# latteine1217/NSFnet

Hardware: AMD Instinct MI355X
Metric: collocation-pt NS-residual evals/sec, Re=2000 6x256 MLP (higher is better)
Workload: dtype bf16x3 (bf16 MFMA, hi/lo split, f32 accumulate)

## Files before the change

nsfnet_amd/csrc/balance.hip:

```cpp
#include <cmath>

#include "kernels.h"

namespace {

constexpr int kBlk = 64;
constexpr int kUpdThreads = 256;

__device__ __forceinline__ void wave_abs_stats(float v, double& mx, double& sm) {
  const double a = fabs((double)v);
  mx = wave_fold<FoldNanMax>(a);
  sm = wave_fold<FoldSum>(a);
}

__global__ __launch_bounds__(512) void reduce_terms_kernel(TermReduceArgs a) {
  __shared__ double part[3][8][64];
  const int H = a.H, HP = a.HP, L = a.L;
  const size_t P = flat_total(H, L, a.n_out);
  const int lane = threadIdx.x & 63, w = threadIdx.x >> 6;
  const size_t p = blockIdx.x * (size_t)64 + lane;
  const bool live = p < P;
  const ReduceLoc loc = live ? reduce_locate(p, H, HP, L, a.n_out) : ReduceLoc{-1, -1, 0};
  const size_t SG = sg_total(HP, L);
  int k = 0;
  for (int t = 0; t < 3; ++t) {
    double s = 0.0;
    for (int j = 0; j < a.nsrc[t]; ++j, ++k)
      if (live) s = reduce_source_add(s, a.src[k], loc, HP, SG, w);
    part[t][w][lane] = s;
  }
  __syncthreads();
  if (w != 0) return;
  float vt[3];
  for (int t = 0; t < 3; ++t) {
    float v = 0.f;
    if (a.out[t] && live) {
      double s = part[t][0][lane];
#pragma unroll
      for (int i = 1; i < 8; ++i) s += part[t][i][lane];
      v = (a.acc_mask >> t) & 1 ? a.out[t][p] + (float)s : (float)s;
      a.out[t][p] = v;
    }
    if (a.partials) {
      double mx, sm;
      wave_abs_stats(v, mx, sm);
      if (lane == 0) {
        a.partials[(size_t)blockIdx.x * 6 + 2 * t] = mx;
        a.partials[(size_t)blockIdx.x * 6 + 2 * t + 1] = sm;
      }
    }
    vt[t] = v;
  }
  if (a.gram) wave_gram(vt[0], vt[1], vt[2], lane, a.gram + (size_t)blockIdx.x * 6);
}

__global__ __launch_bounds__(64) void balance_stats_kernel(const float* __restrict__ v0, const float* __restrict__ v1,
                                                           const float* __restrict__ v2, long n,
                                                           double* __restrict__ partials) {
  const long p = blockIdx.x * (long)kBlk + threadIdx.x;
  const float* v[3] = {v0, v1, v2};
  for (int t = 0; t < 3; ++t) {
    double mx, sm;
    wave_abs_stats(v[t] && p < n ? v[t][p] : 0.f, mx, sm);
    if (threadIdx.x == 0) {
      partials[(size_t)blockIdx.x * 6 + 2 * t] = mx;
      partials[(size_t)blockIdx.x * 6 + 2 * t + 1] = sm;
    }
  }
}

__global__ __launch_bounds__(kUpdThreads) void balance_update_kernel(const double* __restrict__ partials, long nblk,
                                                                     long n, int terms, double beta,
                                                                     float* __restrict__ lam, double* record) {
  __shared__ double red[kUpdThreads][6];
  const int tid = threadIdx.x;
  strided_tree_fold<kUpdThreads, FoldNanMax, FoldSum, FoldNanMax, FoldSum, FoldNanMax, FoldSum>(
      [&](long b, int c) { return partials[b * 6 + c]; }, nblk, red);
  if (tid != 0) return;
  const double P = (double)n;
  const double max_r = red[0][0];
  double rec[12];
  for (int c = 0; c < 12; ++c) rec[c] = record[c];
  rec[0] = max_r; rec[1] = red[0][1] / P;
  for (int t = 1; t < 3; ++t) {
    const int base = 2 + 3 * (t - 1);
    const double mean = red[0][2 * t + 1] / P;
    rec[base] = red[0][2 * t]; rec[base + 1] = mean;
    if (!((terms >> (t - 1)) & 1)) { rec[base + 2] = 0.0; continue; }
    const double lhat = max_r / mean;
    rec[base + 2] = lhat;
    if (mean == 0.0 || !isfinite(lhat)) { rec[8] += 1.0; continue; }
    rec[8 + t] = (1.0 - beta) * rec[8 + t] + beta * lhat;
  }
  rec[11] += 1.0;
  for (int c = 0; c < 12; ++c) record[c] = rec[c];
  lam[0] = (float)rec[9];
  lam[1] = (float)rec[10];
}

__global__ void balance_combine_kernel(float* g, const float* gr, const float* __restrict__ gb,
                                       const float* __restrict__ gs, const float* __restrict__ lam, long n) {
  const float lb = lam[0], ls = gs ? lam[1] : 0.f;
  for (long i = blockIdx.x * (long)blockDim.x + threadIdx.x; i < n; i += (long)gridDim.x * blockDim.x) {
    float v = fmaf(lb, gb[i], gr[i]);
    if (gs) v = fmaf(ls, gs[i], v);
    g[i] = v;
  }
}

}

long balance_blocks(long n) { return (n + kBlk - 1) / kBlk; }

int launch_reduce_terms(const TermReduceArgs& a, hipStream_t s) {
  size_t P = flat_total(a.H, a.L, a.n_out);
  hipLaunchKernelGGL(reduce_terms_kernel, dim3((unsigned)((P + 63) / 64)), dim3(512), 0, s, a);
  return launch_status();
}

int launch_balance_stats(const float* v0, const float* v1, const float* v2, long n, double* partials, hipStream_t s) {
  hipLaunchKernelGGL(balance_stats_kernel, dim3((unsigned)balance_blocks(n)), dim3(kBlk), 0, s, v0, v1, v2, n, partials);
  return launch_status();
}

int launch_balance_update(const double* partials, long n, int terms, double beta, float* lam, double* record,
                          hipStream_t s) {
  hipLaunchKernelGGL(balance_update_kernel, dim3(1), dim3(kUpdThreads), 0, s, partials, balance_blocks(n), n, terms,
                     beta, lam, record);
  return launch_status();
}

int launch_balance_combine(float* g, const float* gr, const float* gb, const float* gs, const float* lam, long n,
                           hipStream_t s) {
  int blocks = (int)((n + 255) / 256);
  if (blocks > 2048) blocks = 2048;
  hipLaunchKernelGGL(balance_combine_kernel, dim3(blocks), dim3(256), 0, s, g, gr, gb, gs, lam, n);
  return launch_status();
}
```

nsfnet_amd/csrc/bwd_bf16_split.hip:

```cpp
#include "kernels.h"
#include "point_stage.h"
#include "split_phases.h"

template <int HP>
struct SplitBwdLds {
  using XI = XImg<HP, 32>;
  static constexpr size_t X_BYTES = XI::BYTES;
  static constexpr size_t OADJ_F = (size_t)2 * 4 * 128;
  static constexpr size_t DUMMY_F = 64 * 8;
  static size_t bytes(int L) { return X_BYTES + (OADJ_F + DUMMY_F + 6 * HP + (size_t)sg_total(HP, L)) * sizeof(float); }
};

template <int HP, int TERMS>
__global__ __launch_bounds__(2 * HP, 1) void bwd_split_kernel(BwdArgs a) {
  using G = SplitBwdLds<HP>;
  using SW = SplitWave<HP, TERMS>;
  constexpr int GT = HP, PPL = SW::PPL, COLS = SW::COLS;
  extern __shared__ __attribute__((aligned(16))) unsigned char ldsb[];
  float* const oadjL = reinterpret_cast<float*>(ldsb + G::X_BYTES);
  float* const dummy = oadjL + G::OADJ_F;
  float* const woutL = dummy + G::DUMMY_F;
  float* const w0L = woutL + 3 * HP;
  float* const sgacc = w0L + 3 * HP;
  const int tid = threadIdx.x, lane0 = tid & 63;
  const int wave = __builtin_amdgcn_readfirstlane(tid >> 6);
  const int grp = wave >> 2, w = wave & 3;
  const int gtid = tid - grp * GT;
  const float* __restrict__ P = a.prep;
  const int L = a.L;
  const int npad = a.ntiles * PPL;
  const int SG = sg_total(HP, L);
  float* const oadjG = oadjL + (size_t)grp * 4 * 128;
  for (int i = tid; i < SG; i += 2 * GT) sgacc[i] = 0.f;
  for (int i = tid; i < 3 * HP; i += 2 * GT) { woutL[i] = P[prep_wout(HP, L) + i]; w0L[i] = P[prep_w0x(HP) + i]; }
  for (int i = tid; i < (int)G::DUMMY_F; i += 2 * GT) dummy[i] = 0.f;
  float dbo[3] = {0.f, 0.f, 0.f};
  SW sw(ldsb, P, woutL, w0L, w, lane0);

  auto S_of = [&](int tile, int l) { return a.S + spill_off<act_block(HP, COLS)>(a.spill, tile < a.ntiles ? tile : 0, l, L); };
  auto Z_of = [&](int tile, int l) { return a.Zb + spill_off<act_block(HP, COLS)>(a.spill, tile, l, L); };
  auto seeds = [&](int tile, float& px, float& py) {
    const int col = lane0 & 31;
    if (tile < a.ntiles) {
      float pxa[1], pya[1];
      output_adjoint_stage<PPL, COLS, 4, GT, 1>(a, tile, gtid, col, col, npad, oadjG, dbo, pxa, pya);
      px = pxa[0]; py = pya[0];
    } else {
      for (int i = gtid; i < 3 * COLS; i += GT) oadjG[i] = 0.f;
      px = py = 0.f;
    }
  };
  auto oadj = [&](int col, int, float (&oc)[3][4]) {
#pragma unroll
    for (int c = 0; c < 3; ++c)
#pragma unroll
      for (int s = 0; s < 4; ++s) oc[c][s] = oadjG[c * COLS + s * PPL + col];
  };
  auto none = [](auto&&...) {};

  const int npairs = (a.ntiles + 1) / 2;
  float px = 0.f, py = 0.f, pxN = 0.f, pyN = 0.f;
  if ((int)blockIdx.x < npairs) seeds(2 * (int)blockIdx.x + grp, px, py);
  __syncthreads();
  if (grp == 1) SW::idle();
  for (int pair = blockIdx.x; pair < npairs; pair += gridDim.x) {
    const int tile = 2 * pair + grp;
    const int next_tile = pair + (int)gridDim.x < npairs ? 2 * (pair + (int)gridDim.x) + grp : -1;
    sw.template bphase<0, false>(L - 1, L, S_of(tile, L - 1), Z_of(tile, L - 1), px, py, sgacc, dummy + wave * 64, oadj, none);
    for (int l = L - 1; l >= 2; --l) {
      sw.template mphase<true, true>(l, S_of(tile, l - 1));
      sw.template bphase<1, false>(l - 1, L, S_of(tile, l - 1), Z_of(tile, l - 1), px, py, sgacc, dummy + wave * 64, oadj, none);
    }
    sw.template mphase<true, false>(1, nullptr);
    sw.template bphase<2, false>(0, L, S_of(tile, 0), Z_of(tile, 0), px, py, sgacc, dummy + wave * 64, oadj,
                                 [&](int q) { if (q == 3 && next_tile >= 0) seeds(next_tile, pxN, pyN); });
    px = pxN; py = pyN;
  }
  if (grp == 0) SW::idle();
  float* red = reinterpret_cast<float*>(ldsb);
  __syncthreads();
#pragma unroll
  for (int c = 0; c < 3; ++c) red[c * 2 * GT + tid] = dbo[c];
  __syncthreads();
  if (tid < 3) {
    float s = 0.f;
    for (int t = 0; t < 2 * GT; ++t) s += red[tid * 2 * GT + t];
    sgacc[sg_bout(HP, L) + tid] = s;
  }
  __syncthreads();
  float* out = a.sg + (size_t)blockIdx.x * SG;
  for (int i = tid; i < SG; i += 2 * GT) out[i] = sgacc[i];
}

size_t bwd_split_lds_bytes(int HP, int L) { (void)HP; return SplitBwdLds<256>::bytes(L); }

template <int HP, int TERMS>
static int launch_one(const BwdArgs& a, int grid, hipStream_t s) {
  const size_t lds = SplitBwdLds<HP>::bytes(a.L);
  if (!spill_is(a.spill, act_block(HP), IN_P24_COMPACT)) return -1000;
  return launch_or_configure(&bwd_split_kernel<HP, TERMS>, dim3(grid), dim3(2 * HP), lds, s, a.configure, a);
}

int launch_bwd_split(int HP, int terms, const BwdArgs& a, int grid, hipStream_t s) {
  if (HP != 256) return -1000;
  return terms == 3 ? launch_one<256, 3>(a, grid, s) : launch_one<256, 1>(a, grid, s);
}
```

nsfnet_amd/csrc/capi.hip:

```cpp
#include <cmath>
#include <cstdio>
#include <cstring>
#include <cstdlib>
#include <new>

#include "../../include/nsfnet_pinn.h"
#include "kernels.h"
#include "optim.h"
#include "rwf.h"

static_assert((int)PINN_FLD_COUNT == (int)FLD_COUNT, "field plane enum mismatch");

static thread_local char g_err[512] = "";
static int fail(int code, const char* fmt, const char* a = "", long b = 0) {
  snprintf(g_err, sizeof(g_err), fmt, a, b);
  return code;
}
static int hipfail(int rc, const char* what) {
  if (rc == -1000) return fail(-22, "%s: unsupported hidden width or spill layout (code %ld)", what, (long)rc);
  return fail(rc, "%s: HIP error %ld", what, (long)-rc);
}

struct Switches {
  int sched_f, sched_b;
  int wsplit, fuse;
  int stagger;
  int s0_skip32;
  int verbose;
  int tile_cols;
};
static int env_int(const char* name, int dflt) {
  const char* v = getenv(name);
  return v ? atoi(v) : dflt;
}
static Switches read_switches() {
  const int sched = env_int("PINN_SCHED", 2);
  return {env_int("PINN_FWD_SCHED", sched), env_int("PINN_BWD_SCHED", sched), env_int("PINN_WSPLIT", 1),
          env_int("PINN_FUSE", 1), env_int("PINN_STAGGER", 0), env_int("PINN_S0_SKIP32", 1),
          env_int("PINN_VERBOSE", 0), env_int("PINN_TILE_COLS", 0)};
}

struct pinn_net_s {
  int n_out, L, H, HP;
  int wide;
  int prec_fwd, prec_bwd, prec_dw;
};
static int terms_of(int prec) { return prec == 1 ? 3 : 1; }
static int pick_wide(const pinn_net_s* n) {
  if (n->HP > 256) return 1;
  if (n->HP != 256 && n->HP != 128) return 0;
  const bool fp32 = !n->prec_fwd && !n->prec_bwd && !n->prec_dw;
  const int force = read_switches().tile_cols;
  if (force == 64) return 1;
  if (force == 128) return 0;
  return fp32 && n->HP == 256;
}

enum Family { FAM_NONE = 0, FAM_FP32, FAM_FP32_WIDE, FAM_BF16, FAM_BF16_WIDE, FAM_PIPE, FAM_SPLIT, FAM_WSPLIT, FAM_FUSED };
static constexpr const char* FAMILY_NAMES[][3] = {
    {nullptr, nullptr, nullptr},
    {"fwd_kernel", "bwd_kernel", "dw_kernel"},
    {"fwd_wide_kernel", "bwd_wide_kernel", "dw_wide_kernel"},
    {"fwd_bf16_kernel", "bwd_bf16_kernel", "dw_bf16_kernel"},
    {"fwd_bf16_wide_kernel", "bwd_bf16_wide_kernel", "dw_bf16_wide_kernel"},
    {"fwd_pipe_kernel", "bwd_pipe_kernel", nullptr},
    {"fwd_split_kernel", "bwd_split_kernel", nullptr},
    {"fwd_wsplit_kernel", "bwd_wsplit_kernel", nullptr},
    {"fwdbwd_split_kernel", "fwdbwd_split_kernel", nullptr},
};
static constexpr unsigned FAMILY_SPILLS[][3] = {
    {0, 0, 0},
    {IN_CLASSIC | IN_SKIP0, IN_CLASSIC | IN_SKIP0, IN_CLASSIC | IN_SKIP0},
    {IN_CLASSIC | IN_SKIP0, IN_CLASSIC | IN_SKIP0, IN_CLASSIC | IN_SKIP0},
    {IN_CLASSIC, IN_CLASSIC, IN_CLASSIC | IN_P24_COMPACT},
    {IN_CLASSIC | IN_P24_WIDE, IN_CLASSIC | IN_P24_WIDE, IN_CLASSIC | IN_P24_WIDE},
    {IN_CLASSIC, IN_CLASSIC, 0},
    {IN_P24_COMPACT, IN_P24_COMPACT, 0},
    {IN_P24_WIDE, IN_P24_WIDE, 0},
    {IN_P24_COMPACT, IN_P24_COMPACT, 0},
};
static Family base_family(const pinn_net_s& n, int prec) {
  return prec ? (n.HP > 256 ? FAM_BF16_WIDE : FAM_BF16) : n.wide ? FAM_FP32_WIDE : FAM_FP32;
}

enum { ROLE_FWD_SAVE = 0, ROLE_FWD, ROLE_BWD, ROLE_DW, ROLE_FUSED, ROLE_COUNT };
static constexpr int ROLE_SPILL_COL[ROLE_COUNT] = {0, -1, 1, 2, 0};
struct Role {
  Family family;
  int grid;
  size_t lds;
  const char* name;
};

struct pinn_plan_s {
  pinn_net_s net;
  long n;
  int streams, ntiles, npad;
  int groups;
  int stagger;
  Role role[ROLE_COUNT];
  Spill spill;
  HardBc hbc;
  size_t off_partials, off_oadj, off_sg, off_slabs, off_S, off_Zb, bytes_fwd, bytes_all;
};

static int num_cus() {
  int dev = 0, n = 0;
  if (hipGetDevice(&dev) == hipSuccess &&
      hipDeviceGetAttribute(&n, hipDeviceAttributeMultiprocessorCount, dev) == hipSuccess && n > 0)
    return n;
  (void)hipGetLastError();
  return 256;
}

static size_t align_up(size_t v, size_t a) { return (v + a - 1) / a * a; }

static size_t fwd_lds(Family f, const pinn_net_s& n) {
  switch (f) {
    case FAM_FP32: return fwd_lds_bytes(n.HP);
    case FAM_FP32_WIDE: return fwd_wide_lds_bytes(n.HP);
    case FAM_BF16: return fwd_bf16_lds_bytes(n.HP, n.L, n.wide ? 64 : 128);
    case FAM_BF16_WIDE: return fwd_bf16_wide_lds_bytes(n.HP, n.L);
    case FAM_PIPE: return fwd_pipe_lds_bytes(n.HP, n.L);
    case FAM_SPLIT: return fwd_split_lds_bytes(n.HP, n.L);
    case FAM_WSPLIT: return fwd_wsplit_lds_bytes(n.HP);
    default: return 0;
  }
}
static size_t bwd_lds(Family f, const pinn_net_s& n) {
  switch (f) {
    case FAM_FP32: return bwd_lds_bytes(n.HP, n.L);
    case FAM_FP32_WIDE: return bwd_wide_lds_bytes(n.HP, n.L);
    case FAM_BF16: return bwd_bf16_lds_bytes(n.HP, n.L, n.wide ? 64 : 128);
    case FAM_BF16_WIDE: return bwd_bf16_wide_lds_bytes(n.HP, n.L);
    case FAM_PIPE: return bwd_pipe_lds_bytes(n.HP, n.L);
    case FAM_SPLIT: return bwd_split_lds_bytes(n.HP, n.L);
    case FAM_WSPLIT: return bwd_wsplit_lds_bytes(n.HP, n.L);
    default: return 0;
  }
}
static size_t dw_lds(Family f, const pinn_net_s& n) {
  switch (f) {
    case FAM_FP32: return dw_lds_bytes(n.HP);
    case FAM_FP32_WIDE: return dw_wide_lds_bytes();
    case FAM_BF16: return dw_bf16_lds_bytes(n.HP);
    case FAM_BF16_WIDE: return dw_bf16_wide_lds_bytes();
    default: return 0;
  }
}
static int run_fwd(const pinn_plan_s* plan, const Role& r, const FwdArgs& a, hipStream_t s) {
  const pinn_net_s& n = plan->net;
  const int NS = plan->streams, terms = terms_of(n.prec_fwd);
  switch (r.family) {
    case FAM_FP32: return launch_fwd(n.HP, NS, a, r.grid, s);
    case FAM_FP32_WIDE: return launch_fwd_wide(n.HP, NS, a, r.grid, s);
    case FAM_BF16: return launch_fwd_bf16(n.HP, NS, terms, n.wide ? 64 : 128, a, r.grid, s);
    case FAM_BF16_WIDE: return launch_fwd_bf16_wide(n.HP, NS, terms, a, r.grid, s);
    case FAM_PIPE: return launch_fwd_pipe(n.HP, terms, a, r.grid, s);
    case FAM_SPLIT: return launch_fwd_split(n.HP, terms, a, r.grid, s);
    case FAM_WSPLIT: return launch_fwd_wsplit(n.HP, terms, a, r.grid, s);
    default: return -1000;
  }
}
static int run_bwd(const pinn_plan_s* plan, const BwdArgs& a, hipStream_t s) {
  const pinn_net_s& n = plan->net;
  const Role& r = plan->role[ROLE_BWD];
  const int NS = plan->streams, terms = terms_of(n.prec_bwd);
  switch (r.family) {
    case FAM_FP32: return launch_bwd(n.HP, NS, a, r.grid, s);
    case FAM_FP32_WIDE: return launch_bwd_wide(n.HP, NS, a, r.grid, s);
    case FAM_BF16: return launch_bwd_bf16(n.HP, NS, terms, n.wide ? 64 : 128, a, r.grid, s);
    case FAM_BF16_WIDE: return launch_bwd_bf16_wide(n.HP, NS, terms, a, r.grid, s);
    case FAM_PIPE: return launch_bwd_pipe(n.HP, terms, a, r.grid, s);
    case FAM_SPLIT: return launch_bwd_split(n.HP, terms, a, r.grid, s);
    case FAM_WSPLIT: return launch_bwd_wsplit(n.HP, terms, a, r.grid, s);
    default: return -1000;
  }
}
static int run_dw(const pinn_plan_s* plan, const DwArgs& d, hipStream_t s) {
  const pinn_net_s& n = plan->net;
  const int NS = plan->streams, terms = terms_of(n.prec_dw);
  switch (plan->role[ROLE_DW].family) {
    case FAM_FP32: return launch_dw(n.HP, NS, d, s);
    case FAM_FP32_WIDE: return launch_dw_wide(n.HP, NS, d, s);
    case FAM_BF16: return launch_dw_bf16(n.HP, NS, terms, n.wide ? 64 : 128, d, s);
    case FAM_BF16_WIDE: return launch_dw_bf16_wide(n.HP, NS, terms, d, s);
    default: return -1000;
  }
}
static int run_fused(const pinn_plan_s* plan, const FwdArgs& fa, const BwdArgs& ba, hipStream_t s) {
  return launch_fwdbwd_split(plan->net.HP, terms_of(plan->net.prec_fwd), fa, ba, plan->role[ROLE_FUSED].grid, s);
}

static int resolve_plan(pinn_plan_s* p, const pinn_net_s& net, long n_points, int streams, int cus, const Switches& sw_in,
                        const HardBc& hbc = HardBc{}) {
  Switches sw = sw_in;
  if (hbc.kind) { sw.sched_f = sw.sched_b = 0; sw.wsplit = 0; sw.fuse = 0; }
  p->net = net;
  p->hbc = hbc;
  p->n = n_points; p->streams = streams;
  const bool wide = net.wide != 0;
  const int per_tile = wide ? (streams == 4 ? 16 : 64) : (streams == 4 ? 32 : 128);
  p->ntiles = (int)((n_points + per_tile - 1) / per_tile);
  p->npad = p->ntiles * per_tile;
  const int HP = net.HP, L = net.L, NW = HP / 32;
  auto bpc = [&](size_t lds) {
    int b = (int)(PINN_LDS_MAX / lds);
    int bw = NW >= 8 ? (wide && NW == 8 ? 2 : 1) : 8 / NW;
    if (b > bw) b = bw;
    return b < 1 ? 1 : b;
  };
  auto role = [&](int which, Family f, int grid, size_t lds, int name_col) {
    p->role[which] = Role{f, grid, lds, FAMILY_NAMES[f][name_col]};
  };
  const Family f8 = base_family(net, net.prec_fwd), b8 = base_family(net, net.prec_bwd), d8 = base_family(net, net.prec_dw);
  const size_t lds_f = fwd_lds(f8, net), lds_b = bwd_lds(b8, net), lds_d = dw_lds(d8, net);
  if (lds_b > PINN_LDS_MAX || lds_f > PINN_LDS_MAX) return fail(-22, "pinn_plan_create: this depth x width needs more than 160 KiB of LDS%s");
  int grid_f = cus * bpc(lds_f);
  if (grid_f > p->ntiles) grid_f = p->ntiles;
  int grid_b = cus * bpc(lds_b);
  if (grid_b > p->ntiles) grid_b = p->ntiles;
  const int grid_fp = cus < (p->ntiles + 1) / 2 ? cus : (p->ntiles + 1) / 2;
  const bool pipe_shape = HP == 256 && !wide && streams == 4 && L >= 2;
  int sf = sw.sched_f, sb = sw.sched_b;
  if (!pipe_shape || !net.prec_fwd) sf = 0;
  if (!pipe_shape || !net.prec_bwd) sb = 0;
  if (sf == 2 && fwd_lds(FAM_SPLIT, net) > PINN_LDS_MAX) sf = 1;
  if (sf == 1 && fwd_lds(FAM_PIPE, net) > PINN_LDS_MAX) sf = 0;
  if (sb == 2 && bwd_lds(FAM_SPLIT, net) > PINN_LDS_MAX) sb = 1;
  if (sb == 1 && bwd_lds(FAM_PIPE, net) > PINN_LDS_MAX) sb = 0;
  if (sf < 0 || sf > 2) sf = 0;
  if (sb < 0 || sb > 2) sb = 0;
  const bool split_pair = sf == 2 && sb == 2 && net.prec_dw;
  if (!split_pair) { if (sf == 2) sf = 1; if (sb == 2) sb = 1; }
  const bool s24w = HP > 256 && streams == 4 && net.prec_fwd && net.prec_bwd && net.prec_dw;
  const bool wsplit = s24w && L >= 2 && sw.wsplit != 0 && fwd_lds(FAM_WSPLIT, net) <= PINN_LDS_MAX &&
                      bwd_lds(FAM_WSPLIT, net) <= PINN_LDS_MAX;
  const bool fuse = sf == 2 && sb == 2 && split_pair && net.prec_fwd == net.prec_bwd && sw.fuse != 0 &&
                    fwdbwd_split_lds_bytes(HP, L) <= PINN_LDS_MAX;
  p->stagger = sw.stagger;
  if (sw.verbose)
    fprintf(stderr, "[pinn] plan: %ld pts, %d streams, HP %d, L %d, prec %d/%d/%d, wide %d, schedule fwd %d bwd %d\n",
            (long)n_points, streams, HP, L, net.prec_fwd, net.prec_bwd, net.prec_dw, (int)wide, sf, sb);
  if (sw.verbose && hbc.kind)
    fprintf(stderr, "[pinn] plan: hard wall conditions, lid-driven cavity at (%g, %g) x %g, lift power %d, lid sharpness %g\n",
            (double)hbc.x0, (double)hbc.y0, (double)hbc.inv_len, hbc.m, (double)hbc.r);
  const Family fs = wsplit ? FAM_WSPLIT : sf == 2 ? FAM_SPLIT : sf == 1 ? FAM_PIPE : f8;
  const Family bs = wsplit ? FAM_WSPLIT : sb == 2 ? FAM_SPLIT : sb == 1 ? FAM_PIPE : b8;
  role(ROLE_FWD, f8, grid_f, lds_f, 0);
  role(ROLE_FWD_SAVE, fs, fs == f8 ? grid_f : grid_fp, fwd_lds(fs, net), 0);
  role(ROLE_BWD, bs, bs == b8 ? grid_b : grid_fp, bwd_lds(bs, net), 1);
  role(ROLE_FUSED, fuse ? FAM_FUSED : FAM_NONE, grid_fp, fuse ? fwdbwd_split_lds_bytes(HP, L) : 0, 0);
  if (L > 1) {
    int g = cus * bpc(lds_d) / (L - 1);
    if (g < 1) g = 1;
    if (g > p->ntiles) g = p->ntiles;
    p->groups = g;
  } else {
    p->groups = 0;
  }
  role(ROLE_DW, d8, p->groups, lds_d, 2);
  const int grid_part = p->role[ROLE_FWD].grid > p->role[ROLE_FWD_SAVE].grid ? p->role[ROLE_FWD].grid : p->role[ROLE_FWD_SAVE].grid;
  size_t off = 0;
  p->off_partials = off; off = align_up(off + (size_t)grid_part * PINN_NLOSS * 4, 256);
  p->off_oadj = off;     off = align_up(off + (size_t)4 * p->npad * 4, 256);
  p->bytes_fwd = off;
  p->off_sg = off;       off = align_up(off + (size_t)p->role[ROLE_BWD].grid * sg_total(HP, L) * 4, 256);
  p->off_slabs = off;    off = align_up(off + (size_t)(L - 1) * p->groups * HP * HP * 4, 256);
  const size_t ablk = act_block(HP, wide ? 64 : PINN_TILE_COLS);
  const bool skip32 = streams == 4 && L >= 2 && !net.prec_fwd && !net.prec_bwd && !net.prec_dw && sw.s0_skip32 != 0;
  p->spill = spill_make(split_pair ? SPILL_P24_COMPACT : s24w ? SPILL_P24_WIDE : skip32 ? SPILL_SKIP0 : SPILL_CLASSIC, ablk);
  for (int r = 0; r < ROLE_COUNT; ++r)
    if (ROLE_SPILL_COL[r] >= 0 && p->role[r].family && (r != ROLE_DW || p->groups) &&
        !spill_is(p->spill, ablk, FAMILY_SPILLS[p->role[r].family][ROLE_SPILL_COL[r]]))
      return fail(-5, "pinn_plan_create: internal error: %s does not implement the plan's spill layout", p->role[r].name);
  const size_t spill_tile = spill_tile_floats(p->spill, L);
  p->off_S = off;        off = align_up(off + (size_t)(p->ntiles + 1) * spill_tile * 4, 256);
  p->off_Zb = off;       off = align_up(off + (size_t)(p->ntiles + 1) * spill_tile * 4, 256);
  p->bytes_all = off;
  return 0;
}

static float* ws_at(void* ws, size_t off) { return ws ? reinterpret_cast<float*>(reinterpret_cast<char*>(ws) + off) : nullptr; }
#define WS(p, off) ws_at(ws, (p)->off)

static FwdArgs fwd_args(const pinn_plan_s* plan, void* ws, const float* prep, const float* x, const float* y, int save, float scale) {
  FwdArgs a;
  memset(&a, 0, sizeof(a));
  a.x = x; a.y = y; a.n = (int)plan->n; a.ntiles = plan->ntiles; a.L = plan->net.L; a.n_out = plan->net.n_out;
  a.prep = prep; a.S = save ? WS(plan, off_S) : nullptr;
  a.scale = scale;
  a.partials = WS(plan, off_partials);
  a.spill = plan->spill;
  a.hbc = plan->hbc;
  return a;
}
static FwdArgs residual_fwd_args(const pinn_plan_s* plan, void* ws, const float* prep, const float* x, const float* y,
                                 const float* e, const float* w, float* vis_t_minus, float* vis_t_out, float* fields,
                                 float Re, float vis_t0, float alpha_evm, float coord_scale, int save, bool stagger) {
  FwdArgs a = fwd_args(plan, ws, prep, x, y, save, coord_scale);
  a.fld = fields; a.e = e; a.w = w; a.vtm = vis_t_minus; a.vis_used = vis_t_out;
  a.inv_re = 1.0f / Re; a.vis_t0 = vis_t0; a.alpha_evm = alpha_evm;
  a.stagger = stagger && plan->ntiles > 4 * plan->role[ROLE_FWD].grid ? plan->stagger : 0;
  return a;
}
static BwdArgs bwd_args(const pinn_plan_s* plan, void* ws, const float* prep, const float* x, const float* y, float scale) {
  BwdArgs a;
  memset(&a, 0, sizeof(a));
  a.x = x; a.y = y; a.n = (int)plan->n; a.ntiles = plan->ntiles; a.L = plan->net.L; a.n_out = plan->net.n_out;
  a.prep = prep; a.S = WS(plan, off_S); a.Zb = WS(plan, off_Zb);
  a.scale = scale;
  a.sg = WS(plan, off_sg);
  a.spill = plan->spill;
  a.hbc = plan->hbc;
  return a;
}
static BwdArgs residual_bwd_args(const pinn_plan_s* plan, void* ws, const float* prep, const float* x, const float* y,
                                 const float* e, const float* w, const float* vis_t, const float* fields,
                                 const float* coef_eq4, float Re, float coord_scale, float* ebar_out) {
  BwdArgs a = bwd_args(plan, ws, prep, x, y, coord_scale);
  a.fld = fields; a.e = e; a.w = w; a.vis_used = vis_t;
  for (int k = 0; k < 4; ++k) a.coef_eq[k] = coef_eq4[k];
  a.inv_re = 1.0f / Re; a.ebar = ebar_out;
  return a;
}
static DwArgs dw_args(const pinn_plan_s* plan, void* ws, const float* prep, const float* x, const float* y) {
  DwArgs d;
  memset(&d, 0, sizeof(d));
  d.S = WS(plan, off_S); d.Zb = WS(plan, off_Zb);
  d.ntiles = plan->ntiles; d.L = plan->net.L; d.groups = plan->groups;
  d.slabs = WS(plan, off_slabs);
  d.x = x; d.y = y; d.prep = prep; d.n = (int)plan->n;
  d.spill = plan->spill;
  return d;
}

static int configure_plan(const pinn_plan_s* p) {
  FwdArgs fa = fwd_args(p, nullptr, nullptr, nullptr, nullptr, 0, 1.f);
  BwdArgs ba = bwd_args(p, nullptr, nullptr, nullptr, nullptr, 1.f);
  DwArgs da = dw_args(p, nullptr, nullptr, nullptr, nullptr);
  fa.configure = ba.configure = da.configure = 1;
  int rc = run_fwd(p, p->role[ROLE_FWD], fa, nullptr);
  if (!rc && p->role[ROLE_FWD_SAVE].family != p->role[ROLE_FWD].family) rc = run_fwd(p, p->role[ROLE_FWD_SAVE], fa, nullptr);
  if (!rc) rc = run_bwd(p, ba, nullptr);
  if (!rc && p->role[ROLE_FUSED].family) rc = run_fused(p, fa, ba, nullptr);
  if (!rc) rc = run_dw(p, da, nullptr);
  return rc;
}

extern "C" {

const char* pinn_last_error(void) { return g_err; }
int pinn_abi_version(void) { return 3; }

int pinn_net_create(int n_out, int n_hidden_layers, int hidden, pinn_net_t* out) {
  if (!out) return fail(-22, "pinn_net_create: null out%s");
  if (n_out < 1 || n_out > 3) return fail(-22, "pinn_net_create: n_out must be 1..3%s");
  if (n_hidden_layers < 1 || n_hidden_layers > 64) return fail(-22, "pinn_net_create: hidden layers must be 1..64%s");
  if (hidden < 1 || hidden > PINN_MAX_HP) return fail(-22, "pinn_net_create: hidden width must be 1..512 (got %s%ld)", "", hidden);
  pinn_net_s* n = new (std::nothrow) pinn_net_s;
  if (!n) return fail(-12, "pinn_net_create: out of host memory%s");
  n->n_out = n_out; n->L = n_hidden_layers; n->H = hidden; n->HP = (hidden + 31) / 32 * 32;
  n->prec_fwd = n->prec_bwd = n->prec_dw = 0;
  n->wide = pick_wide(n);
  *out = n;
  return 0;
}
int pinn_net_set_precision(pinn_net_t net, int prec_fwd, int prec_bwd, int prec_dw) {
  if (!net) return fail(-22, "pinn_net_set_precision: null net%s");
  if (prec_fwd < 0 || prec_fwd > 2 || prec_bwd < 0 || prec_bwd > 2 || prec_dw < 0 || prec_dw > 2)
    return fail(-22, "pinn_net_set_precision: precision must be 0 (fp32), 1 (bf16x3) or 2 (bf16)%s");
  net->prec_fwd = prec_fwd; net->prec_bwd = prec_bwd; net->prec_dw = prec_dw;
  net->wide = pick_wide(net);
  return 0;
}
int pinn_net_destroy(pinn_net_t net) { delete net; return 0; }
int64_t pinn_net_num_params(pinn_net_t net) { return net ? (int64_t)flat_total(net->H, net->L, net->n_out) : -1; }
int64_t pinn_net_prep_floats(pinn_net_t net) { return net ? (int64_t)prep_total(net->HP, net->L) : -1; }

int pinn_net_prepare(pinn_net_t net, const float* params, float* prep, void* stream) {
  if (!net || !params || !prep) return fail(-22, "pinn_net_prepare: null argument%s");
  int rc = launch_prep(params, prep, net->H, net->HP, net->L, net->n_out, net->prec_fwd, net->prec_bwd,
                       (hipStream_t)stream);
  return rc ? hipfail(rc, "pinn_net_prepare") : 0;
}

static int create_plan(pinn_net_t net, int64_t n_points, int streams, const HardBc& hbc, pinn_plan_t* out) {
  if (!net || !out) return fail(-22, "pinn_plan_create: null argument%s");
  if (streams != 1 && streams != 4) return fail(-22, "pinn_plan_create: streams must be 1 or 4%s");
  if (n_points < 1 || n_points > (int64_t)1 << 30) return fail(-22, "pinn_plan_create: bad point count %s%ld", "", (long)n_points);
  pinn_plan_s* p = new (std::nothrow) pinn_plan_s;
  if (!p) return fail(-12, "pinn_plan_create: out of host memory%s");
  int rc = resolve_plan(p, *net, (long)n_points, streams, num_cus(), read_switches(), hbc);
  if (rc) { delete p; return rc; }
  int ndev = 0;
  if (hipGetDeviceCount(&ndev) != hipSuccess) { ndev = 0; (void)hipGetLastError(); }
  if (ndev > 0) {
    rc = configure_plan(p);
    if (rc) { delete p; return hipfail(rc, "pinn_plan_create(kernel attributes)"); }
  }
  *out = p;
  return 0;
}
int pinn_plan_create(pinn_net_t net, int64_t n_points, int streams, pinn_plan_t* out) {
  return create_plan(net, n_points, streams, HardBc{}, out);
}
int pinn_plan_create_constrained(pinn_net_t net, int64_t n_points, int streams, const pinn_hard_bc_t* bc, pinn_plan_t* out) {
  if (!bc || bc->kind == PINN_HARD_BC_NONE) return pinn_plan_create(net, n_points, streams, out);
  if (!net || !out) return fail(-22, "pinn_plan_create_constrained: null argument%s");
  if (bc->kind != PINN_HARD_BC_CAVITY) return fail(-22, "pinn_plan_create_constrained: unknown kind %s%ld", "", (long)bc->kind);
  if (net->n_out != 3) return fail(-22, "pinn_plan_create_constrained: only a (u, v, p) net (n_out = 3) can be constrained%s");
  if (bc->lift_power < 1 || bc->lift_power > 8)
    return fail(-22, "pinn_plan_create_constrained: lift_power must be 1..8 (got %s%ld)", "", (long)bc->lift_power);
  if (!std::isfinite(bc->x0) || !std::isfinite(bc->y0) || !std::isfinite(bc->inv_len) || !std::isfinite(bc->lid_sharpness))
    return fail(-22, "pinn_plan_create_constrained: x0, y0, inv_len and lid_sharpness must be finite%s");
  if (!(bc->inv_len > 0.f)) return fail(-22, "pinn_plan_create_constrained: inv_len must be > 0%s");
  if (std::fabs(bc->lid_sharpness) > 150.f)
    return fail(-22, "pinn_plan_create_constrained: |lid_sharpness| must be <= 150%s");
  HardBc h;
  h.kind = bc->kind; h.m = bc->lift_power; h.x0 = bc->x0; h.y0 = bc->y0; h.inv_len = bc->inv_len; h.r = bc->lid_sharpness;
  h.c = (float)(1.0 / std::cosh(0.5 * (double)bc->lid_sharpness));
  return create_plan(net, n_points, streams, h, out);
}
int pinn_plan_hard_bc(pinn_plan_t plan, pinn_hard_bc_t* out) {
  if (!plan || !out) return fail(-22, "pinn_plan_hard_bc: null argument%s");
  const HardBc& h = plan->hbc;
  out->kind = h.kind; out->lift_power = h.m; out->x0 = h.x0; out->y0 = h.y0; out->inv_len = h.inv_len; out->lid_sharpness = h.r;
  return 0;
}
int pinn_plan_destroy(pinn_plan_t plan) { delete plan; return 0; }
int64_t pinn_plan_padded_points(pinn_plan_t plan) { return plan ? plan->npad : -1; }
const char* pinn_plan_kernel(pinn_plan_t plan, int which) {
  if (!plan || which < 0 || which > 2) return nullptr;
  return plan->role[which == 0 ? ROLE_FWD_SAVE : which == 1 ? ROLE_BWD : ROLE_DW].name;
}
int64_t pinn_plan_workspace_bytes(pinn_plan_t plan, int with_backward) {
  if (!plan) return -1;
  return (int64_t)(with_backward ? plan->bytes_all : plan->bytes_fwd);
}

static int check_hard_bc_scale(const char* what, const pinn_plan_s* plan, float coord_scale) {
  if (plan->hbc.kind && !(std::fabs((double)coord_scale * (double)plan->hbc.inv_len - 1.0) <= 1e-6))
    return fail(-22, "%s: coord_scale x inv_len of the plan's hard wall conditions must be 1", what);
  return 0;
}

static int run_loss_sums(const Role& r, const FwdArgs& a, float* loss_sums, hipStream_t s, const char* what) {
  if (!loss_sums) return 0;
  int rc = launch_loss_sums(a.partials, r.grid, loss_sums, s);
  return rc ? hipfail(rc, what) : 0;
}

int pinn_residual_forward(pinn_plan_t plan, void* ws, const float* prep,
                          const float* x, const float* y, const float* e, const float* w,
                          float* vis_t_minus, float* vis_t_out, float* fields,
                          float Re, float vis_t0, float alpha_evm, float coord_scale,
                          int save, float* loss_sums, void* stream) {
  if (!plan || !ws || !prep || !x || !y || !fields) return fail(-22, "pinn_residual_forward: null argument%s");
  if (plan->streams != 4) return fail(-22, "pinn_residual_forward: plan is not a residual (4-stream) plan%s");
  if (!(Re > 0.f)) return fail(-22, "pinn_residual_forward: Re must be > 0%s");
  if (int rc = check_hard_bc_scale("pinn_residual_forward", plan, coord_scale)) return rc;
  const FwdArgs a = residual_fwd_args(plan, ws, prep, x, y, e, w, vis_t_minus, vis_t_out, fields, Re, vis_t0, alpha_evm,
                                      coord_scale, save, true);
  const Role& r = plan->role[save ? ROLE_FWD_SAVE : ROLE_FWD];
  int rc = run_fwd(plan, r, a, (hipStream_t)stream);
  if (rc) return hipfail(rc, "pinn_residual_forward");
  return run_loss_sums(r, a, loss_sums, (hipStream_t)stream, "pinn_residual_forward(loss sums)");
}

static int run_dw_and_stash(pinn_plan_t plan, void* ws, const float* prep, const float* x, const float* y, hipStream_t s) {
  return run_dw(plan, dw_args(plan, ws, prep, x, y), s);
}

int pinn_residual_backward_phases(pinn_plan_t plan, void* ws, const float* prep,
                                  const float* x, const float* y, const float* e, const float* w,
                                  const float* vis_t, const float* fields, const float* coef_eq4,
                                  float Re, float coord_scale, float* ebar_out, int phases, void* stream) {
  if (!plan || !ws || !prep || !x || !y || !fields || !coef_eq4) return fail(-22, "pinn_residual_backward: null argument%s");
  if (plan->streams != 4) return fail(-22, "pinn_residual_backward: plan is not a residual (4-stream) plan%s");
  if (int rc = check_hard_bc_scale("pinn_residual_backward", plan, coord_scale)) return rc;
  const BwdArgs a = residual_bwd_args(plan, ws, prep, x, y, e, w, vis_t, fields, coef_eq4, Re, coord_scale, ebar_out);
  int rc = 0;
  if (phases & 1) {
    rc = run_bwd(plan, a, (hipStream_t)stream);
    if (rc) return hipfail(rc, "pinn_residual_backward");
  }
  if (phases & 2) rc = run_dw_and_stash(plan, ws, prep, x, y, (hipStream_t)stream);
  return rc ? hipfail(rc, "pinn_residual_backward(dW)") : 0;
}

int pinn_residual_backward(pinn_plan_t plan, void* ws, const float* prep,
                           const float* x, const float* y, const float* e, const float* w,
                           const float* vis_t, const float* fields, const float* coef_eq4,
                           float Re, float coord_scale, float* ebar_out, void* stream) {
  return pinn_residual_backward_phases(plan, ws, prep, x, y, e, w, vis_t, fields, coef_eq4, Re, coord_scale,
                                       ebar_out, 3, stream);
}

int pinn_residual_forward_backward(pinn_plan_t plan, void* ws, const float* prep,
                                   const float* x, const float* y, const float* e, const float* w,
                                   float* vis_t_minus, float* vis_t_out, float* fields,
                                   const float* coef_eq4, float Re, float vis_t0, float alpha_evm,
                                   float coord_scale, float* loss_sums, float* ebar_out, void* stream) {
  if (!plan || !ws || !prep || !x || !y || !fields || !coef_eq4) return fail(-22, "pinn_residual_forward_backward: null argument%s");
  if (plan->streams != 4) return fail(-22, "pinn_residual_forward_backward: plan is not a residual (4-stream) plan%s");
  if (!plan->role[ROLE_FUSED].family) {
    int rc = pinn_residual_forward(plan, ws, prep, x, y, e, w, vis_t_minus, vis_t_out, fields, Re, vis_t0, alpha_evm,
                                   coord_scale, 1, loss_sums, stream);
    return rc ? rc : pinn_residual_backward(plan, ws, prep, x, y, e, w, vis_t_out, fields, coef_eq4, Re, coord_scale,
                                            ebar_out, stream);
  }
  if (!(Re > 0.f)) return fail(-22, "pinn_residual_forward_backward: Re must be > 0%s");
  const FwdArgs fa = residual_fwd_args(plan, ws, prep, x, y, e, w, vis_t_minus, vis_t_out, fields, Re, vis_t0, alpha_evm,
                                       coord_scale, 1, false);
  const BwdArgs a = residual_bwd_args(plan, ws, prep, x, y, e, w, vis_t_out, fields, coef_eq4, Re, coord_scale, ebar_out);
  hipStream_t s = (hipStream_t)stream;
  int rc = run_fused(plan, fa, a, s);
  if (rc) return hipfail(rc, "pinn_residual_forward_backward");
  rc = run_loss_sums(plan->role[ROLE_FUSED], fa, loss_sums, s, "pinn_residual_forward_backward(loss sums)");
  if (rc) return rc;
  rc = run_dw_and_stash(plan, ws, prep, x, y, s);
  return rc ? hipfail(rc, "pinn_residual_forward_backward(dW)") : 0;
}

int pinn_value_forward(pinn_plan_t plan, void* ws, const float* prep,
                       const float* x, const float* y,
                       float* const* pred3, const float* const* tgt3, const float* coef3,
                       int save, float* loss_sums, void* stream) {
  if (!plan || !ws || !prep || !x || !y) return fail(-22, "pinn_value_forward: null argument%s");
  if (plan->streams != 1) return fail(-22, "pinn_value_forward: plan is not a value (1-stream) plan%s");
  FwdArgs a = fwd_args(plan, ws, prep, x, y, save, 1.f);
  for (int c = 0; c < 3; ++c) {
    a.pred[c] = (pred3 && c < a.n_out) ? pred3[c] : nullptr;
    a.tgt[c] = (tgt3 && c < a.n_out) ? tgt3[c] : nullptr;
    a.coef[c] = coef3 ? coef3[c] : 0.f;
  }
  a.oadj = save ? WS(plan, off_oadj) : nullptr;
  const Role& r = plan->role[ROLE_FWD];
  int rc = run_fwd(plan, r, a, (hipStream_t)stream);
  if (rc) return hipfail(rc, "pinn_value_forward");
  return run_loss_sums(r, a, loss_sums, (hipStream_t)stream, "pinn_value_forward(loss sums)");
}

int pinn_value_backward(pinn_plan_t plan, void* ws, const float* prep,
                        const float* x, const float* y, const float* out_adj, void* stream) {
  if (!plan || !ws || !prep || !x || !y) return fail(-22, "pinn_value_backward: null argument%s");
  if (plan->streams != 1) return fail(-22, "pinn_value_backward: plan is not a value (1-stream) plan%s");
  BwdArgs a = bwd_args(plan, ws, prep, x, y, 1.f);
  a.oadj = out_adj ? out_adj : WS(plan, off_oadj);
  int rc = run_bwd(plan, a, (hipStream_t)stream);
  if (rc) return hipfail(rc, "pinn_value_backward");
  rc = run_dw_and_stash(plan, ws, prep, x, y, (hipStream_t)stream);
  return rc ? hipfail(rc, "pinn_value_backward(dW)") : 0;
}

static int reduce_sources(const char* who, const pinn_net_s* net, int nsrc, const pinn_plan_t* plans, void* const* wss,
                          ReduceSrc* src) {
  for (int k = 0; k < nsrc; ++k) {
    pinn_plan_t p = plans[k];
    void* ws = wss[k];
    if (!p || !ws) return fail(-22, "%s: null plan/workspace", who);
    if (p->net.H != net->H || p->net.L != net->L || p->net.n_out != net->n_out)
      return fail(-22, "%s: plan belongs to a different net", who);
    src[k].slabs = WS(p, off_slabs); src[k].groups = p->groups;
    src[k].sg = WS(p, off_sg); src[k].nwg = p->role[ROLE_BWD].grid;
  }
  return 0;
}

int pinn_grad_reduce(pinn_net_t net, int nsrc, const pinn_plan_t* plans, void* const* wss,
                     float* grads, int accumulate, void* stream) {
  if (!net || !plans || !wss || !grads) return fail(-22, "pinn_grad_reduce: null argument%s");
  if (nsrc < 1 || nsrc > 4) return fail(-22, "pinn_grad_reduce: nsrc must be 1..4%s");
  ReduceArgs r;
  memset(&r, 0, sizeof(r));
  r.nsrc = nsrc; r.H = net->H; r.HP = net->HP; r.L = net->L; r.n_out = net->n_out;
  r.grads = grads; r.accumulate = accumulate;
  if (int rc = reduce_sources("pinn_grad_reduce", net, nsrc, plans, wss, r.src)) return rc;
  int rc = launch_reduce(r, (hipStream_t)stream);
  return rc ? hipfail(rc, "pinn_grad_reduce") : 0;
}

int pinn_adam_step(float* params, const float* grads, float* m, float* v, int64_t n,
                   float lr, float beta1, float beta2, float eps, int64_t step, void* stream) {
  if (!params || !grads || !m || !v) return fail(-22, "pinn_adam_step: null argument%s");
  if (step < 1) return fail(-22, "pinn_adam_step: step must be >= 1%s");
  double bc1 = 1.0 - std::pow((double)beta1, (double)step);
  double bc2 = 1.0 - std::pow((double)beta2, (double)step);
  int rc = launch_adam(params, grads, m, v, (long)n, (float)((double)lr / bc1), beta1, beta2, eps, (float)std::sqrt(bc2),
                       (hipStream_t)stream);
  return rc ? hipfail(rc, "pinn_adam_step") : 0;
}

int pinn_adam_step_dev(float* params, const float* grads, float* m, float* v, int64_t n,
                       float lr, float beta1, float beta2, float eps, int64_t* step_counter, void* stream) {
  if (!params || !grads || !m || !v || !step_counter) return fail(-22, "pinn_adam_step_dev: null argument%s");
  int rc = launch_adam_dev(params, grads, m, v, (long)n, lr, beta1, beta2, eps,
                           reinterpret_cast<long long*>(step_counter), (hipStream_t)stream);
  return rc ? hipfail(rc, "pinn_adam_step_dev") : 0;
}

int64_t pinn_resample_scratch_bytes(int64_t n_pool) {
  return n_pool < 1 || n_pool > (int64_t)1 << 30 ? -1 : (int64_t)resample_scratch_bytes((long)n_pool);
}

int pinn_resample_select(int64_t n_pool, const float* fields, int64_t npad, double w4, double k, double c,
                         double u, int64_t m, void* scratch, int64_t* out, void* stream) {
  if (!fields || !scratch || !out) return fail(-22, "pinn_resample_select: null argument%s");
  if (n_pool < 1 || n_pool > (int64_t)1 << 30) return fail(-22, "pinn_resample_select: pool size must be 1..2^30 (got %s%ld)", "", (long)n_pool);
  if (m < 1 || m > (int64_t)1 << 30) return fail(-22, "pinn_resample_select: m must be 1..2^30 (got %s%ld)", "", (long)m);
  if (npad < n_pool || npad % 4 != 0) return fail(-22, "pinn_resample_select: npad must be >= n_pool and a multiple of 4%s");
  if (reinterpret_cast<uintptr_t>(fields) % 16 != 0) return fail(-22, "pinn_resample_select: fields must be 16-byte aligned%s");
  if (!std::isfinite(k) || k < 0.0) return fail(-22, "pinn_resample_select: k must be finite and >= 0%s");
  if (!std::isfinite(c) || c < 0.0) return fail(-22, "pinn_resample_select: c must be finite and >= 0%s");
  if (!std::isfinite(w4) || w4 < 0.0) return fail(-22, "pinn_resample_select: w4 must be finite and >= 0%s");
  if (!(u >= 0.0 && u < 1.0)) return fail(-22, "pinn_resample_select: u must be in [0, 1)%s");
  int rc = launch_resample_select((long)n_pool, fields, (long)npad, w4, k, c, u, (long)m, scratch,
                                  reinterpret_cast<long long*>(out), (hipStream_t)stream);
  return rc ? hipfail(rc, "pinn_resample_select") : 0;
}

int pinn_resample_gather(const int64_t* idx, int64_t lo, int64_t hi, int64_t n_pool,
                         const float* src_x, const float* src_y, const float* src_w, const float* src_vtm,
                         float* dst_x, float* dst_y, float* dst_w, float* dst_vtm,
                         void* scratch, double* w_sum, void* stream) {
  if (!idx || !src_x || !src_y || !dst_x || !dst_y || !scratch) return fail(-22, "pinn_resample_gather: null argument%s");
  if (n_pool < 1 || n_pool > (int64_t)1 << 30) return fail(-22, "pinn_resample_gather: pool size must be 1..2^30 (got %s%ld)", "", (long)n_pool);
  if (lo < 0 || hi <= lo) return fail(-22, "pinn_resample_gather: need 0 <= lo < hi%s");
  if (!src_w != !dst_w) return fail(-22, "pinn_resample_gather: src_w and dst_w must both be given or both be NULL%s");
  if (!src_vtm != !dst_vtm) return fail(-22, "pinn_resample_gather: src_vtm and dst_vtm must both be given or both be NULL%s");
  if (w_sum && !dst_w) return fail(-22, "pinn_resample_gather: w_sum needs the weights%s");
  int rc = launch_resample_gather(reinterpret_cast<const long long*>(idx), (long)lo, (long)hi, (long)n_pool, src_x, src_y,
                                  src_w, src_vtm, dst_x, dst_y, dst_w, dst_vtm, scratch, w_sum, (hipStream_t)stream);
  return rc ? hipfail(rc, "pinn_resample_gather") : 0;
}

int64_t pinn_lbfgs_workspace_bytes(int64_t n, int history) {
  if (n < 1 || n > (int64_t)1 << 30 || history < 1 || history > PINN_LBFGS_MAX_HISTORY) return -1;
  return (int64_t)lbfgs_workspace_bytes((long)n, (long)history);
}

static int lbfgs_args(const char* what, void* ws, int64_t n, int history) {
  if (!ws) return fail(-22, "%s: null workspace", what);
  if (n < 1 || n > (int64_t)1 << 30) return fail(-22, "%s: n must be 1..2^30", what);
  if (history < 1 || history > PINN_LBFGS_MAX_HISTORY) return fail(-22, "%s: history must be 1..1024", what);
  if (reinterpret_cast<uintptr_t>(ws) % 256 != 0) return fail(-22, "%s: workspace must be 256-byte aligned", what);
  return 0;
}

int pinn_lbfgs_reset(void* ws, int64_t n, int history, void* stream) {
  if (int rc = lbfgs_args("pinn_lbfgs_reset", ws, n, history)) return rc;
  int rc = launch_lbfgs_reset(ws, (long)n, history, (hipStream_t)stream);
  return rc ? hipfail(rc, "pinn_lbfgs_reset") : 0;
}

int pinn_lbfgs_direction(void* ws, int64_t n, int history, const float* g, float t_prev, float* d, double* result,
                         void* stream) {
  if (int rc = lbfgs_args("pinn_lbfgs_direction", ws, n, history)) return rc;
  if (!g || !d || !result) return fail(-22, "pinn_lbfgs_direction: null argument%s");
  if (reinterpret_cast<uintptr_t>(g) % 16 != 0 || reinterpret_cast<uintptr_t>(d) % 16 != 0)
    return fail(-22, "pinn_lbfgs_direction: g and d must be 16-byte aligned%s");
  if (!std::isfinite(t_prev)) return fail(-22, "pinn_lbfgs_direction: t_prev must be finite%s");
  int rc = launch_lbfgs_direction(ws, (long)n, history, g, t_prev, d, result, (hipStream_t)stream);
  return rc ? hipfail(rc, "pinn_lbfgs_direction") : 0;
}

int pinn_lbfgs_probe(void* ws, int64_t n, int history, const float* g, const float* d, double* result, void* stream) {
  if (int rc = lbfgs_args("pinn_lbfgs_probe", ws, n, history)) return rc;
  if (!g || !d || !result) return fail(-22, "pinn_lbfgs_probe: null argument%s");
  if (reinterpret_cast<uintptr_t>(g) % 16 != 0 || reinterpret_cast<uintptr_t>(d) % 16 != 0)
    return fail(-22, "pinn_lbfgs_probe: g and d must be 16-byte aligned%s");
  int rc = launch_lbfgs_probe(ws, (long)n, history, g, d, result, (hipStream_t)stream);
  return rc ? hipfail(rc, "pinn_lbfgs_probe") : 0;
}

int64_t pinn_balance_partials_count(int64_t n) {
  return n < 1 || n > (int64_t)1 << 30 ? -1 : (int64_t)balance_blocks((long)n) * 6;
}

static int reduce_terms(const char* what, pinn_net_t net, const int* nsrc3, const pinn_plan_t* plans, void* const* wss,
                        float* const* out3, int accumulate_mask, double* partials, double* gram, void* stream) {
  if (!net || !nsrc3 || !out3) return fail(-22, "%s: null argument", what);
  TermReduceArgs r;
  memset(&r, 0, sizeof(r));
  int total = 0;
  for (int t = 0; t < 3; ++t) {
    if (nsrc3[t] < 0) return fail(-22, "%s: negative source count", what);
    if (nsrc3[t] > 0 && !out3[t]) return fail(-22, "%s: a group with sources needs its output", what);
    r.nsrc[t] = nsrc3[t]; r.out[t] = out3[t];
    total += nsrc3[t];
  }
  if (total < 1 || total > 4) return fail(-22, "%s: 1..4 sources in all", what);
  if (!plans || !wss) return fail(-22, "%s: null argument", what);
  r.H = net->H; r.HP = net->HP; r.L = net->L; r.n_out = net->n_out;
  r.acc_mask = accumulate_mask & 7; r.partials = partials; r.gram = gram;
  if (int rc = reduce_sources(what, net, total, plans, wss, r.src)) return rc;
  int rc = launch_reduce_terms(r, (hipStream_t)stream);
  return rc ? hipfail(rc, what) : 0;
}

int pinn_grad_reduce_terms(pinn_net_t net, const int* nsrc3, const pinn_plan_t* plans, void* const* wss,
                           float* const* out3, int accumulate_mask, double* partials, void* stream) {
  return reduce_terms("pinn_grad_reduce_terms", net, nsrc3, plans, wss, out3, accumulate_mask, partials, nullptr, stream);
}

int pinn_grad_reduce_terms_gram(pinn_net_t net, const int* nsrc3, const pinn_plan_t* plans, void* const* wss,
                                float* const* out3, int accumulate_mask, double* partials, double* gram_partials,
                                void* stream) {
  return reduce_terms("pinn_grad_reduce_terms_gram", net, nsrc3, plans, wss, out3, accumulate_mask, partials,
                      gram_partials, stream);
}

int pinn_balance_stats(const float* const* vec3, int64_t n, double* partials, void* stream) {
  if (!vec3 || !partials) return fail(-22, "pinn_balance_stats: null argument%s");
  if (n < 1 || n > (int64_t)1 << 30) return fail(-22, "pinn_balance_stats: n must be 1..2^30%s");
  int rc = launch_balance_stats(vec3[0], vec3[1], vec3[2], (long)n, partials, (hipStream_t)stream);
  return rc ? hipfail(rc, "pinn_balance_stats") : 0;
}

int pinn_balance_update(const double* partials, int64_t n, int terms, double beta, float* lam, double* record,
                        void* stream) {
  if (!partials || !lam || !record) return fail(-22, "pinn_balance_update: null argument%s");
  if (n < 1 || n > (int64_t)1 << 30) return fail(-22, "pinn_balance_update: n must be 1..2^30%s");
  if (terms < 0 || terms > 3) return fail(-22, "pinn_balance_update: terms must be 0..3%s");
  if (!(beta > 0.0 && beta <= 1.0)) return fail(-22, "pinn_balance_update: beta must be in (0, 1]%s");
  int rc = launch_balance_update(partials, (long)n, terms, beta, lam, record, (hipStream_t)stream);
  return rc ? hipfail(rc, "pinn_balance_update") : 0;
}

int pinn_balance_combine(float* g, const float* gr, const float* gb, const float* gs, const float* lam, int64_t n,
                         void* stream) {
  if (!g || !gr || !gb || !lam) return fail(-22, "pinn_balance_combine: null argument%s");
  if (n < 1 || n > (int64_t)1 << 30) return fail(-22, "pinn_balance_combine: n must be 1..2^30%s");
  int rc = launch_balance_combine(g, gr, gb, gs, lam, (long)n, (hipStream_t)stream);
  return rc ? hipfail(rc, "pinn_balance_combine") : 0;
}

int64_t pinn_confgrad_partials_count(int64_t n) { return pinn_balance_partials_count(n); }

int pinn_confgrad_gram(const float* const* vec3, int64_t n, double* partials, void* stream) {
  if (!vec3 || !partials) return fail(-22, "pinn_confgrad_gram: null argument%s");
  if (n < 1 || n > (int64_t)1 << 30) return fail(-22, "pinn_confgrad_gram: n must be 1..2^30%s");
  int rc = launch_confgrad_gram(vec3[0], vec3[1], vec3[2], (long)n, partials, (hipStream_t)stream);
  return rc ? hipfail(rc, "pinn_confgrad_gram") : 0;
}

int pinn_confgrad_coef(const double* partials, int64_t n, int nterms, float* coef, double* record, void* stream) {
  if (!partials || !coef || !record) return fail(-22, "pinn_confgrad_coef: null argument%s");
  if (n < 1 || n > (int64_t)1 << 30) return fail(-22, "pinn_confgrad_coef: n must be 1..2^30%s");
  if (nterms < 2 || nterms > 3) return fail(-22, "pinn_confgrad_coef: nterms must be 2 or 3%s");
  int rc = launch_confgrad_coef(partials, (long)n, nterms, coef, record, (hipStream_t)stream);
  return rc ? hipfail(rc, "pinn_confgrad_coef") : 0;
}

int pinn_confgrad_combine(float* g, const float* gr, const float* gb, const float* gs, const float* coef, int64_t n,
                          void* stream) {
  if (!g || !gr || !gb || !coef) return fail(-22, "pinn_confgrad_combine: null argument%s");
  if (n < 1 || n > (int64_t)1 << 30) return fail(-22, "pinn_confgrad_combine: n must be 1..2^30%s");
  int rc = launch_confgrad_combine(g, gr, gb, gs, coef, (long)n, (hipStream_t)stream);
  return rc ? hipfail(rc, "pinn_confgrad_combine") : 0;
}

int pinn_batch_draw(int64_t n, int64_t b, uint64_t seed, int rank, int64_t* counter,
                    const float* src_x, const float* src_y, const float* src_w, const float* src_vtm,
                    float* dst_x, float* dst_y, float* dst_w, float* dst_vtm, int64_t* idx, void* stream) {
  if (!counter || !src_x || !src_y || !dst_x || !dst_y || !idx) return fail(-22, "pinn_batch_draw: null argument%s");
  if (n < 1 || n > (int64_t)1 << 30) return fail(-22, "pinn_batch_draw: store size must be 1..2^30 (got %s%ld)", "", (long)n);
  if (b < 1 || b > n) return fail(-22, "pinn_batch_draw: batch size must be 1..n (got %s%ld)", "", (long)b);
  if (rank < 0) return fail(-22, "pinn_batch_draw: rank must be >= 0%s");
  if (!src_w != !dst_w) return fail(-22, "pinn_batch_draw: src_w and dst_w must both be given or both be NULL%s");
  if (!src_vtm != !dst_vtm) return fail(-22, "pinn_batch_draw: src_vtm and dst_vtm must both be given or both be NULL%s");
  BatchDrawArgs a;
  a.n = (long)n; a.b = (long)b;
  a.seed = (unsigned)(seed & 0xffffffffu); a.rank = (unsigned)rank;
  a.counter = reinterpret_cast<long long*>(counter);
  a.sx = src_x; a.sy = src_y; a.sw = src_w; a.sv = src_vtm;
  a.dx = dst_x; a.dy = dst_y; a.dw = dst_w; a.dv = dst_vtm;
  a.idx = reinterpret_cast<long long*>(idx);
  int rc = launch_batch_draw(a, (hipStream_t)stream);
  return rc ? hipfail(rc, "pinn_batch_draw") : 0;
}

int pinn_batch_scatter(const int64_t* idx, int64_t b, int64_t n, const float* batch_vtm, float* store_vtm,
                       void* stream) {
  if (!idx || !batch_vtm || !store_vtm) return fail(-22, "pinn_batch_scatter: null argument%s");
  if (n < 1 || n > (int64_t)1 << 30) return fail(-22, "pinn_batch_scatter: store size must be 1..2^30 (got %s%ld)", "", (long)n);
  if (b < 1 || b > n) return fail(-22, "pinn_batch_scatter: batch size must be 1..n (got %s%ld)", "", (long)b);
  int rc = launch_batch_scatter(reinterpret_cast<const long long*>(idx), (long)b, (long)n, batch_vtm, store_vtm,
                                (hipStream_t)stream);
  return rc ? hipfail(rc, "pinn_batch_scatter") : 0;
}

int64_t pinn_rba_scratch_bytes(int64_t n) {
  return n < 1 || n > (int64_t)1 << 30 ? -1 : (int64_t)rba_scratch_bytes((long)n);
}

static int rba_planes(const char* what, int64_t n, const float* fields, int64_t npad, double w4) {
  if (n < 1 || n > (int64_t)1 << 30) return fail(-22, "%s: n must be 1..2^30 (got %ld)", what, (long)n);
  if (!fields) return fail(-22, "%s: null field planes", what);
  if (npad < n || npad % 4 != 0) return fail(-22, "%s: npad must be >= n and a multiple of 4", what);
  if (reinterpret_cast<uintptr_t>(fields) % 16 != 0) return fail(-22, "%s: fields must be 16-byte aligned", what);
  if (!std::isfinite(w4) || w4 < 0.0) return fail(-22, "%s: w4 must be finite and >= 0", what);
  return 0;
}

int pinn_rba_stats(int64_t n, const float* fields, int64_t npad, double w4, double* scratch, void* stream) {
  if (int rc = rba_planes("pinn_rba_stats", n, fields, npad, w4)) return rc;
  if (!scratch || reinterpret_cast<uintptr_t>(scratch) % 8 != 0) return fail(-22, "pinn_rba_stats: scratch must be given and 8-byte aligned%s");
  int rc = launch_rba_stats((long)n, fields, (long)npad, w4, scratch, (hipStream_t)stream);
  return rc ? hipfail(rc, "pinn_rba_stats") : 0;
}

int pinn_rba_apply(int64_t n, const float* fields, int64_t npad, double w4, double gamma, double eta,
                   const int64_t* idx, int64_t n_store, const float* s, float* lam, float* w, double* scratch,
                   double* record, void* stream) {
  if (int rc = rba_planes("pinn_rba_apply", n, fields, npad, w4)) return rc;
  if (!lam || !w || !scratch || !record) return fail(-22, "pinn_rba_apply: null argument%s");
  if (reinterpret_cast<uintptr_t>(scratch) % 8 != 0) return fail(-22, "pinn_rba_apply: scratch must be 8-byte aligned%s");
  if (n_store < 1 || n_store > (int64_t)1 << 30) return fail(-22, "pinn_rba_apply: store size must be 1..2^30 (got %s%ld)", "", (long)n_store);
  if (!idx && n > n_store) return fail(-22, "pinn_rba_apply: without idx n must be <= n_store%s");
  if (!(gamma > 0.0 && gamma <= 1.0)) return fail(-22, "pinn_rba_apply: gamma must be in (0, 1]%s");
  if (!std::isfinite(eta) || eta < 0.0) return fail(-22, "pinn_rba_apply: eta must be finite and >= 0%s");
  if (reinterpret_cast<uintptr_t>(lam) % 16 != 0 || reinterpret_cast<uintptr_t>(w) % 16 != 0 ||
      reinterpret_cast<uintptr_t>(s) % 16 != 0)
    return fail(-22, "pinn_rba_apply: s, lam and w must be 16-byte aligned%s");
  if (lam == w || s == lam || s == w) return fail(-22, "pinn_rba_apply: s, lam and w must be distinct buffers%s");
  RbaApplyArgs a;
  a.n = (long)n; a.npad = (long)npad; a.n_store = (long)n_store;
  a.fld = fields; a.w4 = w4; a.gamma = gamma; a.eta = eta;
  a.idx = reinterpret_cast<const long long*>(idx);
  a.s = s; a.lam = lam; a.w = w; a.scratch = scratch; a.record = record;
  int rc = launch_rba_apply(a, (hipStream_t)stream);
  return rc ? hipfail(rc, "pinn_rba_apply") : 0;
}

int pinn_rba_fill(int64_t n, double init, const float* s, float* lam, float* w, void* stream) {
  if (!lam || !w) return fail(-22, "pinn_rba_fill: null argument%s");
  if (n < 1 || n > (int64_t)1 << 30) return fail(-22, "pinn_rba_fill: n must be 1..2^30 (got %s%ld)", "", (long)n);
  if (!std::isfinite(init) || init < 0.0) return fail(-22, "pinn_rba_fill: init must be finite and >= 0%s");
  int rc = launch_rba_fill((long)n, init, s, lam, w, (hipStream_t)stream);
  return rc ? hipfail(rc, "pinn_rba_fill") : 0;
}

static int check_schedule(const char* what, const pinn_lr_schedule_t* s) {
  if (!s) return fail(-22, "%s: null schedule", what);
  if (s->kind < PINN_LR_CONSTANT || s->kind > PINN_LR_COSINE) return fail(-22, "%s: unknown schedule kind %ld", what, (long)s->kind);
  if (s->warmup_epochs < 0) return fail(-22, "%s: warmup_epochs must be >= 0", what);
  if (s->warmup_epochs > 0 && !(s->warmup_start >= 0.0 && s->warmup_start <= 1.0))
    return fail(-22, "%s: warmup_start must be in [0, 1]", what);
  if (s->kind == PINN_LR_CONSTANT) return 0;
  if (s->kind == PINN_LR_COSINE) {
    if (s->t_max < 1) return fail(-22, "%s: t_max must be >= 1", what);
    if (!std::isfinite(s->eta_min)) return fail(-22, "%s: eta_min must be finite", what);
    return 0;
  }
  if (!(s->gamma > 0.0) || !std::isfinite(s->gamma)) return fail(-22, "%s: gamma must be finite and > 0", what);
  if (s->kind == PINN_LR_STEP && s->step_size < 1) return fail(-22, "%s: step_size must be >= 1", what);
  if (s->kind == PINN_LR_MULTISTEP) {
    if (s->n_milestones < 0 || s->n_milestones > PINN_LR_MAX_MILESTONES)
      return fail(-22, "%s: at most 16 milestones (got %ld)", what, (long)s->n_milestones);
    for (int i = 0; i < s->n_milestones; ++i)
      if (s->milestones[i] < 0 || (i > 0 && s->milestones[i] < s->milestones[i - 1]))
        return fail(-22, "%s: milestones must be >= 0 and non-decreasing", what);
  }
  return 0;
}

double pinn_lr_schedule_value(const pinn_lr_schedule_t* schedule, double lr0, int64_t e) {
  if (check_schedule("pinn_lr_schedule_value", schedule)) return NAN;
  if (e < 0) { fail(-22, "pinn_lr_schedule_value: e must be >= 0%s"); return NAN; }
  return lr_schedule_value(*schedule, lr0, (long long)e);
}

int64_t pinn_grad_sqnorm_scratch_bytes(void) { return (int64_t)grad_sqnorm_scratch_bytes(); }

int pinn_grad_sqnorm(const float* g0, int64_t n0, const float* g1, int64_t n1, double* scratch, void* stream) {
  if (!g0 || !scratch) return fail(-22, "pinn_grad_sqnorm: null argument%s");
  if (n0 < 1 || n0 > (int64_t)1 << 30) return fail(-22, "pinn_grad_sqnorm: n0 must be 1..2^30 (got %s%ld)", "", (long)n0);
  if (n1 < 0 || n1 > (int64_t)1 << 30) return fail(-22, "pinn_grad_sqnorm: n1 must be 0..2^30 (got %s%ld)", "", (long)n1);
  if ((n1 > 0) != (g1 != nullptr)) return fail(-22, "pinn_grad_sqnorm: g1 must be given exactly when n1 > 0%s");
  if (reinterpret_cast<uintptr_t>(scratch) % 8 != 0) return fail(-22, "pinn_grad_sqnorm: scratch must be 8-byte aligned%s");
  if (reinterpret_cast<uintptr_t>(g0) % 4 != 0 || reinterpret_cast<uintptr_t>(g1) % 4 != 0)
    return fail(-22, "pinn_grad_sqnorm: the vectors must be 4-byte aligned%s");
  int rc = launch_grad_sqnorm(g0, (long)n0, g1, (long)n1, scratch, (hipStream_t)stream);
  return rc ? hipfail(rc, "pinn_grad_sqnorm") : 0;
}

int pinn_adam_step_sched(float* params, const float* grads, float* m, float* v, int64_t n,
                         const pinn_lr_schedule_t* schedule, double lr0, float beta1, float beta2, float eps,
                         int64_t* step_counter, int64_t* epoch, int advance, const double* sqnorm, double max_norm,
                         double* record, void* stream) {
  if (!params || !grads || !m || !v || !step_counter || !epoch || !record)
    return fail(-22, "pinn_adam_step_sched: null argument%s");
  if (n < 1 || n > (int64_t)1 << 30) return fail(-22, "pinn_adam_step_sched: n must be 1..2^30 (got %s%ld)", "", (long)n);
  if (int rc = check_schedule("pinn_adam_step_sched", schedule)) return rc;
  if (!std::isfinite(lr0)) return fail(-22, "pinn_adam_step_sched: lr0 must be finite%s");
  if (sqnorm && !(max_norm > 0.0)) return fail(-22, "pinn_adam_step_sched: max_norm must be > 0 when sqnorm is given%s");
  if (reinterpret_cast<uintptr_t>(sqnorm) % 8 != 0 || reinterpret_cast<uintptr_t>(record) % 8 != 0 ||
      reinterpret_cast<uintptr_t>(epoch) % 8 != 0)
    return fail(-22, "pinn_adam_step_sched: epoch, sqnorm and record must be 8-byte aligned%s");
  AdamSchedArgs a;
  a.p = params; a.g = grads; a.m = m; a.v = v; a.n = (long)n;
  a.sched = *schedule; a.lr0 = lr0; a.b1 = beta1; a.b2 = beta2; a.eps = eps;
  a.step_counter = reinterpret_cast<long long*>(step_counter);
  a.epoch = reinterpret_cast<long long*>(epoch);
  a.advance = advance != 0; a.sq = sqnorm; a.max_norm = max_norm; a.record = record;
  int rc = launch_adam_sched(a, (hipStream_t)stream);
  return rc ? hipfail(rc, "pinn_adam_step_sched") : 0;
}

static RwfNet rwf_net(const pinn_net_s* net) {
  RwfNet n;
  n.H = net->H; n.L = net->L; n.n_out = net->n_out;
  return n;
}
static bool misaligned4(const void* p) { return reinterpret_cast<uintptr_t>(p) % 4 != 0; }
static bool overlap(const float* a, size_t na, const float* b, size_t nb) {
  const uintptr_t a0 = reinterpret_cast<uintptr_t>(a), b0 = reinterpret_cast<uintptr_t>(b);
  return a0 < b0 + 4 * nb && b0 < a0 + 4 * na;
}

int64_t pinn_rwf_rows(pinn_net_t net) { return net ? (int64_t)rwf_rows(rwf_net(net)) : -1; }

int pinn_rwf_split(pinn_net_t net, const float* params, const float* s, float* theta, void* stream) {
  if (!net || !params || !s || !theta) return fail(-22, "pinn_rwf_split: null argument%s");
  if (misaligned4(params) || misaligned4(s) || misaligned4(theta))
    return fail(-22, "pinn_rwf_split: the vectors must be 4-byte aligned%s");
  const RwfNet n = rwf_net(net);
  const size_t P = flat_total(n.H, n.L, n.n_out), R = (size_t)rwf_rows(n);
  if (overlap(theta, P + R, params, P) || overlap(theta, P + R, s, R))
    return fail(-22, "pinn_rwf_split: theta must not overlap params or s%s");
  int rc = launch_rwf_split(n, params, s, theta, (hipStream_t)stream);
  return rc ? hipfail(rc, "pinn_rwf_split") : 0;
}

int pinn_rwf_compose(pinn_net_t net, const float* theta, float* params, void* stream) {
  if (!net || !theta || !params) return fail(-22, "pinn_rwf_compose: null argument%s");
  if (misaligned4(theta) || misaligned4(params)) return fail(-22, "pinn_rwf_compose: the vectors must be 4-byte aligned%s");
  const RwfNet n = rwf_net(net);
  const size_t P = flat_total(n.H, n.L, n.n_out), R = (size_t)rwf_rows(n);
  if (overlap(theta, P + R, params, P)) return fail(-22, "pinn_rwf_compose: params must not overlap theta%s");
  int rc = launch_rwf_compose(n, theta, params, (hipStream_t)stream);
  return rc ? hipfail(rc, "pinn_rwf_compose") : 0;
}

int pinn_rwf_grad(pinn_net_t net, const float* theta, const float* grads, float* gtheta, void* stream) {
  if (!net || !theta || !grads || !gtheta) return fail(-22, "pinn_rwf_grad: null argument%s");
  if (misaligned4(theta) || misaligned4(grads) || misaligned4(gtheta))
    return fail(-22, "pinn_rwf_grad: the vectors must be 4-byte aligned%s");
  const RwfNet n = rwf_net(net);
  const size_t P = flat_total(n.H, n.L, n.n_out), R = (size_t)rwf_rows(n);
  if (overlap(gtheta, P + R, theta, P + R) || overlap(gtheta, P + R, grads, P))
    return fail(-22, "pinn_rwf_grad: gtheta must not overlap theta or grads%s");
  int rc = launch_rwf_grad(n, theta, grads, gtheta, (hipStream_t)stream);
  return rc ? hipfail(rc, "pinn_rwf_grad") : 0;
}

int64_t pinn_val_scratch_bytes(void) { return (int64_t)val_scratch_bytes(); }

static bool misaligned(const void* p, uintptr_t a) { return reinterpret_cast<uintptr_t>(p) % a != 0; }

int pinn_val_stats(int64_t n, const float* const* pred3, const float* const* tgt3, int metric, double t, int64_t every,
                   double* scratch, double* state, double* ring, int64_t capacity, void* stream) {
  static_assert(PINN_VAL_RECORD == VAL_RECORD && PINN_VAL_STATE == VAL_STATE, "validation record / state size mismatch");
  if (n < 1 || n > (int64_t)1 << 30) return fail(-22, "pinn_val_stats: n must be 1..2^30 (got %s%ld)", "", (long)n);
  if (capacity < 1 || capacity > (int64_t)1 << 30) return fail(-22, "pinn_val_stats: capacity must be 1..2^30 (got %s%ld)", "", (long)capacity);
  if (every < 1) return fail(-22, "pinn_val_stats: every must be >= 1 (got %s%ld)", "", (long)every);
  if (metric < 0 || metric > 4) return fail(-22, "pinn_val_stats: metric must be 0..4 (got %s%ld)", "", (long)metric);
  if (!(t == -1.0 || (t >= 0.0 && std::isfinite(t)))) return fail(-22, "pinn_val_stats: t must be -1 (the cadence) or finite and >= 0%s");
  if (!pred3 || !tgt3 || !scratch || !state || !ring) return fail(-22, "pinn_val_stats: null argument%s");
  if (misaligned(scratch, 8) || misaligned(state, 8) || misaligned(ring, 8))
    return fail(-22, "pinn_val_stats: scratch, state and ring must be 8-byte aligned%s");
  ValStatsArgs a;
  for (int c = 0; c < 3; ++c) {
    a.pred[c] = pred3[c]; a.tgt[c] = tgt3[c];
    if (c < 2 && (!a.pred[c] || !a.tgt[c])) return fail(-22, "pinn_val_stats: the u and v planes must be given%s");
    if (misaligned(a.pred[c], 16) || misaligned(a.tgt[c], 16)) return fail(-22, "pinn_val_stats: every plane must be 16-byte aligned%s");
  }
  if (!a.pred[2] != !a.tgt[2]) return fail(-22, "pinn_val_stats: the pressure prediction and target come together%s");
  if (metric >= 3 && !a.pred[2]) return fail(-22, "pinn_val_stats: a pressure metric needs the pressure planes%s");
  a.n = (long)n; a.capacity = (long)capacity; a.metric = metric; a.t = t; a.every = (double)every;
  a.scratch = scratch; a.state = state; a.ring = ring;
  int rc = launch_val_stats(a, (hipStream_t)stream);
  return rc ? hipfail(rc, "pinn_val_stats") : 0;
}

int pinn_val_keep(const float* src0, float* dst0, int64_t n0, const float* src1, float* dst1, int64_t n1,
                  const double* state, void* stream) {
  if (!src0 || !dst0 || !state) return fail(-22, "pinn_val_keep: null argument%s");
  if (n0 < 1 || n0 > (int64_t)1 << 30) return fail(-22, "pinn_val_keep: n0 must be 1..2^30 (got %s%ld)", "", (long)n0);
  if (n1 < 0 || n1 > (int64_t)1 << 30) return fail(-22, "pinn_val_keep: n1 must be 0..2^30 (got %s%ld)", "", (long)n1);
  if (n1 > 0 && (!src1 || !dst1)) return fail(-22, "pinn_val_keep: the second segment has a length but no buffers%s");
  if (misaligned(src0, 4) || misaligned(dst0, 4) || misaligned(src1, 4) || misaligned(dst1, 4) || misaligned(state, 8))
    return fail(-22, "pinn_val_keep: the segments must be 4-byte aligned, state 8-byte%s");
  ValKeepArgs a;
  a.src[0] = src0; a.dst[0] = dst0; a.n[0] = (long)n0;
  a.src[1] = n1 > 0 ? src1 : nullptr; a.dst[1] = n1 > 0 ? dst1 : nullptr; a.n[1] = (long)n1;
  a.state = state;
  int rc = launch_val_keep(a, (hipStream_t)stream);
  return rc ? hipfail(rc, "pinn_val_keep") : 0;
}

}
```

nsfnet_amd/csrc/dw_bf16.hip:

```cpp
#include "kernels.h"
#include "bf16_util.h"

template <int T> struct DwCfgB;
template <> struct DwCfgB<1> { static constexpr int TM = 1, TN = 1; };
template <> struct DwCfgB<2> { static constexpr int TM = 1, TN = 2; };
template <> struct DwCfgB<3> { static constexpr int TM = 1, TN = 3; };
template <> struct DwCfgB<4> { static constexpr int TM = 2, TN = 2; };
template <> struct DwCfgB<5> { static constexpr int TM = 1, TN = 5; };
template <> struct DwCfgB<6> { static constexpr int TM = 2, TN = 3; };
template <> struct DwCfgB<7> { static constexpr int TM = 1, TN = 7; };
template <> struct DwCfgB<8> { static constexpr int TM = 4, TN = 2; };

template <int HP>
struct DwImg {
  static constexpr int PADB = ((64 - 2 * HP) % 256 + 256) % 256;
  static constexpr int RSB = 2 * HP + PADB;
  static constexpr int CH = 32;
  static constexpr int ARR = CH * RSB;
  static constexpr size_t BYTES = (size_t)2 * 4 * ARR;
};

typedef __attribute__((address_space(3))) unsigned char lds_u8;
__device__ __forceinline__ u32x2 tr_read(const lds_u8* p) {
  typedef __attribute__((address_space(3))) s16x4 lds_s16x4;
  s16x4 v = __builtin_amdgcn_ds_read_tr16_b64_v4i16((lds_s16x4*)(p));
  return __builtin_bit_cast(u32x2, v);
}

template <int HP, int NS, int TERMS, int PPL, bool REC, bool P24>
__device__ __forceinline__ void dw_bf16_body(const DwArgs& a) {
  constexpr int CPT = PPL / 8;
  constexpr size_t ABLK = act_block(HP, 4 * PPL);
  using DI = DwImg<HP>;
  static_assert(P24 || !REC, "no fp32-format reader that recomputes layer 0");
  constexpr int T = HP / 32;
  constexpr int TM = DwCfgB<T>::TM, TN = DwCfgB<T>::TN;
  constexpr int WN = T / TN;
  extern __shared__ __attribute__((aligned(16))) unsigned char ldsb[];
  const int tid = threadIdx.x, lane = tid & 63, i32 = lane & 31, h = lane >> 5;
  const int w = __builtin_amdgcn_readfirstlane(tid >> 6);
  const int wr = w / WN, wc = w % WN;
  const int l = blockIdx.y + 1;
  const int g = blockIdx.x;
  const int t0 = (int)((long)g * a.ntiles / a.groups), t1 = (int)((long)(g + 1) * a.ntiles / a.groups);
  const int nch = (t1 - t0) * CPT;
  const int p = tid & 7, og = tid >> 3;

  f32x16 acc[TM][TN];
#pragma unroll
  for (int m = 0; m < TM; ++m)
#pragma unroll
    for (int n = 0; n < TN; ++n)
#pragma unroll
      for (int r = 0; r < 16; ++r) acc[m][n][r] = 0.f;

  constexpr bool rec = REC;
  f32x4 wx4 = {0.f, 0.f, 0.f, 0.f}, wy4 = wx4, b4 = wx4;
  if (rec) {
    const f32x4* w0 = reinterpret_cast<const f32x4*>(a.prep + prep_w0x(HP));
    wx4 = w0[og]; wy4 = w0[HP / 4 + og]; b4 = w0[2 * (HP / 4) + og];
  }
  f32x4 zrA[4], srA[4];
  struct Raw24 { u32x4 z[3], s[3]; float px, py; };
  Raw24 rawA, rawB;
  auto gload24 = [&](int ch, Raw24& R) {
    const int tile = t0 + ch / CPT, c = ch % CPT;
    const unsigned lo_ = (unsigned)(og * PPL + p);
#ifndef PINN_ABL
#define PINN_ABL 0
#endif
    load_quad24(a.Zb + spill_off<ABLK>(a.spill, ((PINN_ABL & 512) && l == a.L - 1) ? 0 : tile, l, a.L) + 32 * c, (HP / 4) * PPL, lo_, R.z);
    if (rec) {
      const int pt = tile * PPL + 8 * c + p;
      R.px = pt < a.n ? a.x[pt] : 0.f; R.py = pt < a.n ? a.y[pt] : 0.f;
    } else {
      load_quad24(a.S + spill_off<ABLK>(a.spill, tile, l - 1, a.L) + 32 * c, (HP / 4) * PPL, lo_, R.s);
    }
  };
  auto gload = [&](int ch, f32x4 (&zr)[4], f32x4 (&sr)[4]) {
    if (P24) { gload24(ch, rawA); return; }
    const int tile = t0 + ch / CPT, c = ch % CPT;
    const unsigned lo_ = (unsigned)(og * PPL + p);
    const float* Zg = a.Zb + spill_off<ABLK, 0>(a.spill, tile, l, a.L) + 32 * c;
    const float* Sg = a.S + spill_off<ABLK, 0>(a.spill, tile, l - 1, a.L) + 32 * c;
#pragma unroll
    for (int s = 0; s < 4; ++s) { zr[s] = load_plane(Zg, (HP / 4) * PPL, s, lo_); sr[s] = load_plane(Sg, (HP / 4) * PPL, s, lo_); }
  };
  auto lstore_r = [&](int buf, f32x4 (&zr)[4], f32x4 (&sr)[4], const Raw24& R) {
    if (P24) {
#pragma unroll
      for (int s = 0; s < 4; ++s) {
        zr[s] = unpack24(u32x2{R.z[s >> 1][2 * (s & 1)], R.z[s >> 1][2 * (s & 1) + 1]}, R.z[2][s]);
        if (!rec) sr[s] = unpack24(u32x2{R.s[s >> 1][2 * (s & 1)], R.s[s >> 1][2 * (s & 1) + 1]}, R.s[2][s]);
      }
    }
    f32x4 av[4];
    if (rec) {
      const float px = R.px, py = R.py;
#pragma unroll
      for (int e = 0; e < 4; ++e) {
        const float t = layer0_t(wx4[e], wy4[e], b4[e], px, py, TanhFast()), zx = wx4[e], zy = wy4[e];
        const float d1 = 1.f - t * t, d2 = -2.f * t * d1;
        av[0][e] = t; av[1][e] = d1 * zx; av[2][e] = d1 * zy; av[3][e] = d2 * (zx * zx + zy * zy);
      }
    } else if (NS == 4) {
#pragma unroll
      for (int e = 0; e < 4; ++e) {
        float t = sr[0][e], zx = sr[1][e], zy = sr[2][e], zd = sr[3][e];
        float d1 = 1.f - t * t, d2 = -2.f * t * d1;
        av[0][e] = t; av[1][e] = d1 * zx; av[2][e] = d1 * zy; av[3][e] = d2 * (zx * zx + zy * zy) + d1 * zd;
      }
    } else {
      av[0] = sr[0]; av[1] = sr[1]; av[2] = sr[2]; av[3] = sr[3];
    }
    unsigned char* base = ldsb + (size_t)buf * 4 * DI::ARR + p * DI::RSB + (og ^ (p & 6)) * 8;
#pragma unroll
    for (int s = 0; s < 4; ++s) {
      u32x2 hi, lo;
      unsigned char* row = base + s * 8 * DI::RSB;
      split4(zr[s][0], zr[s][1], zr[s][2], zr[s][3], hi, lo);
      *reinterpret_cast<u32x2*>(row + 0 * DI::ARR) = hi;
      if (TERMS == 3) *reinterpret_cast<u32x2*>(row + 1 * DI::ARR) = lo;
      split4(av[s][0], av[s][1], av[s][2], av[s][3], hi, lo);
      *reinterpret_cast<u32x2*>(row + 2 * DI::ARR) = hi;
      if (TERMS == 3) *reinterpret_cast<u32x2*>(row + 3 * DI::ARR) = lo;
    }
  };
  auto lstore = [&](int buf, f32x4 (&zr)[4], f32x4 (&sr)[4]) { lstore_r(buf, zr, sr, rawA); };
  const int li = lane & 15, fb = (lane >> 4) & 1, q = li >> 2, pp = li & 3;
  const int lane_off = (8 * h + q) * DI::RSB + ((4 * fb + pp) ^ (q & 2)) * 8;
  const int lane_off4 = (8 * h + q + 4) * DI::RSB + ((4 * fb + pp) ^ ((q & 2) | 4)) * 8 - lane_off;
  auto mfma_chunk = [&](int buf) {
    const lds_u8* B0 = (const lds_u8*)ldsb + buf * 4 * DI::ARR + lane_off;
#pragma unroll
    for (int ks = 0; ks < DI::CH / 16; ++ks) {
      u32x4 zh[TM], zl[TM], ah[TN], al[TN];
#pragma unroll
      for (int m = 0; m < TM; ++m) {
        const lds_u8* pz = B0 + ks * 16 * DI::RSB + 64 * (wr * TM + m);
        u32x2 x0 = tr_read(pz), x1 = tr_read(pz + lane_off4);
        zh[m][0] = x0[0]; zh[m][1] = x0[1]; zh[m][2] = x1[0]; zh[m][3] = x1[1];
        if (TERMS == 3) {
          u32x2 y0 = tr_read(pz + DI::ARR), y1 = tr_read(pz + DI::ARR + lane_off4);
          zl[m][0] = y0[0]; zl[m][1] = y0[1]; zl[m][2] = y1[0]; zl[m][3] = y1[1];
        }
      }
#pragma unroll
      for (int n = 0; n < TN; ++n) {
        const lds_u8* pa = B0 + 2 * DI::ARR + ks * 16 * DI::RSB + 64 * (wc * TN + n);
        u32x2 x0 = tr_read(pa), x1 = tr_read(pa + lane_off4);
        ah[n][0] = x0[0]; ah[n][1] = x0[1]; ah[n][2] = x1[0]; ah[n][3] = x1[1];
        if (TERMS == 3) {
          u32x2 y0 = tr_read(pa + DI::ARR), y1 = tr_read(pa + DI::ARR + lane_off4);
          al[n][0] = y0[0]; al[n][1] = y0[1]; al[n][2] = y1[0]; al[n][3] = y1[1];
        }
      }
#pragma unroll
      for (int m = 0; m < TM; ++m)
#pragma unroll
        for (int n = 0; n < TN; ++n) {
          if (TERMS == 3) {
            acc[m][n] = MFMA_Q(ks, zh[m], al[n], acc[m][n]);
            acc[m][n] = MFMA_Q(ks + 1, zl[m], ah[n], acc[m][n]);
          }
          acc[m][n] = MFMA_Q(ks, zh[m], ah[n], acc[m][n]);
        }
    }
  };

#ifndef PINN_DWDEPTH
#define PINN_DWDEPTH 1
#endif
  constexpr int NMF = (DI::CH / 16) * TM * TN * (TERMS == 3 ? 3 : 1);
  auto interleave = [&]() {
#pragma unroll
    for (int i = 0; i < NMF; ++i) {
      __builtin_amdgcn_sched_group_barrier(0x008, 1, 0);
      __builtin_amdgcn_sched_group_barrier(0x002, P24 ? 5 : 4, 0);
    }
  };
  if (P24 && PINN_DWDEPTH == 2) {
    if (nch > 0) {
      gload24(0, rawA);
      lstore_r(0, zrA, srA, rawA);
      gload24(nch > 1 ? 1 : 0, rawA);
      gload24(nch > 2 ? 2 : nch - 1, rawB);
    }
    __syncthreads();
    int ch = 0;
    for (; ch + 2 < nch; ch += 2) {
      mfma_chunk(0);
      lstore_r(1, zrA, srA, rawA);
      gload24(ch + 3 < nch ? ch + 3 : nch - 1, rawA);
      interleave();
      __syncthreads();
      mfma_chunk(1);
      lstore_r(0, zrA, srA, rawB);
      gload24(ch + 4 < nch ? ch + 4 : nch - 1, rawB);
      interleave();
      __syncthreads();
    }
    if (ch < nch) mfma_chunk(0);
    if (ch + 1 < nch) {
      lstore_r(1, zrA, srA, rawA);
      __syncthreads();
      mfma_chunk(1);
    }
    __syncthreads();
  } else {
  if (nch > 0) {
    gload(0, zrA, srA);
    lstore(0, zrA, srA);
    if (nch > 1) gload(1, zrA, srA);
  }
  __syncthreads();
  for (int ch = 0; ch + 1 < nch; ++ch) {
    const int buf = ch & 1;
    mfma_chunk(buf);
    lstore(buf ^ 1, zrA, srA);
    gload(ch + 2 < nch ? ch + 2 : nch - 1, zrA, srA);
    interleave();
    __syncthreads();
  }
  if (nch > 0) mfma_chunk((nch - 1) & 1);
  __syncthreads();
  }
  float* slab = a.slabs + ((size_t)(l - 1) * a.groups + g) * HP * HP;
#pragma unroll
  for (int m = 0; m < TM; ++m)
#pragma unroll
    for (int n = 0; n < TN; ++n)
#pragma unroll
      for (int r = 0; r < 16; ++r) {
        int o = 32 * (wr * TM + m) + mfma_row(r, h);
        int i = 32 * (wc * TN + n) + i32;
        slab[(size_t)o * HP + i] = acc[m][n][r];
      }
}

template <int HP, int NS, int TERMS, int PPL, bool P24, bool REC0>
__global__ __launch_bounds__(HP * 2) void dw_bf16_kernel(DwArgs a) {
  if (REC0 && blockIdx.y == 0) dw_bf16_body<HP, NS, TERMS, PPL, REC0, P24>(a);
  else dw_bf16_body<HP, NS, TERMS, PPL, false, P24>(a);
}

template <int HP>
static size_t lds_bytes_t() { return DwImg<HP>::BYTES; }

size_t dw_bf16_lds_bytes(int HP) {
  switch (HP) {
    case 32: return lds_bytes_t<32>(); case 64: return lds_bytes_t<64>(); case 96: return lds_bytes_t<96>();
    case 128: return lds_bytes_t<128>(); case 160: return lds_bytes_t<160>(); case 192: return lds_bytes_t<192>();
    case 224: return lds_bytes_t<224>(); default: return lds_bytes_t<256>();
  }
}

template <int HP, int NS, int TERMS, int PPL, bool P24, bool REC0>
static int launch_fmt(const DwArgs& a, hipStream_t s) {
  size_t lds = lds_bytes_t<HP>();
  return launch_or_configure(&dw_bf16_kernel<HP, NS, TERMS, PPL, P24, REC0>, dim3(a.groups, a.L - 1), dim3(HP * 2), lds, s, a.configure, a);
}
template <int HP, int NS, int TERMS, int PPL>
static int launch_one(const DwArgs& a, hipStream_t s) {
  constexpr bool CAN_COMPACT = HP == 256 && NS == 4 && PPL == 32;
  if (!spill_is(a.spill, act_block(HP, 4 * PPL), CAN_COMPACT ? IN_CLASSIC | IN_P24_COMPACT : IN_CLASSIC)) return -1000;
  const bool p24 = a.spill.quad == SPILL_QUAD_P24, rec0 = a.spill.skip0 != 0;
  if constexpr (CAN_COMPACT) {
    if (p24 && rec0) return launch_fmt<HP, NS, TERMS, PPL, true, true>(a, s);
  }
  return p24 || rec0 ? -1000 : launch_fmt<HP, NS, TERMS, PPL, false, false>(a, s);
}

template <int HP, int PPL>
static int launch_hp(int NS, int terms, const DwArgs& a, hipStream_t s) {
  if (terms == 3) return NS == 4 ? launch_one<HP, 4, 3, PPL>(a, s) : launch_one<HP, 1, 3, PPL>(a, s);
  return NS == 4 ? launch_one<HP, 4, 1, PPL>(a, s) : launch_one<HP, 1, 1, PPL>(a, s);
}

int launch_dw_bf16(int HP, int NS, int terms, int cols, const DwArgs& a, hipStream_t s) {
  if (a.L <= 1 || a.groups <= 0) return 0;
  if (cols == 64) {
    switch (HP) {
      case 128: return launch_hp<128, 16>(NS, terms, a, s);
      case 256: return launch_hp<256, 16>(NS, terms, a, s);
      default: return -1000;
    }
  }
  switch (HP) {
    case 32: return launch_hp<32, 32>(NS, terms, a, s);
    case 64: return launch_hp<64, 32>(NS, terms, a, s);
    case 96: return launch_hp<96, 32>(NS, terms, a, s);
    case 128: return launch_hp<128, 32>(NS, terms, a, s);
    case 160: return launch_hp<160, 32>(NS, terms, a, s);
    case 192: return launch_hp<192, 32>(NS, terms, a, s);
    case 224: return launch_hp<224, 32>(NS, terms, a, s);
    case 256: return launch_hp<256, 32>(NS, terms, a, s);
    default: return -1000;
  }
}
```

nsfnet_amd/csrc/fwdbwd_bf16_split.hip:

```cpp
#include "kernels.h"
#include "split_phases.h"

template <int HP>
struct FusedLds {
  using XI = XImg<HP, 32>;
  static constexpr size_t X_BYTES = XI::BYTES;
  static constexpr size_t PART_F = (size_t)2 * 4 * 12 * 32;
  static size_t bytes(int L) { return X_BYTES + (PART_F + 6 * HP + (size_t)sg_total(HP, L)) * sizeof(float); }
};

template <int HP, int TERMS>
__global__ __launch_bounds__(2 * HP, 1) void fwdbwd_split_kernel(FwdArgs fa, BwdArgs a) {
  using G = FusedLds<HP>;
  using SW = SplitWave<HP, TERMS>;
  constexpr int GT = HP, PPL = SW::PPL, COLS = SW::COLS;
  extern __shared__ __attribute__((aligned(16))) unsigned char ldsb[];
  float* const part = reinterpret_cast<float*>(ldsb + G::X_BYTES);
  float* const woutL = part + G::PART_F;
  float* const w0L = woutL + 3 * HP;
  float* const sgacc = w0L + 3 * HP;
  const int tid = threadIdx.x, lane0 = tid & 63;
  const int wave = __builtin_amdgcn_readfirstlane(tid >> 6);
  const int grp = wave >> 2, w = wave & 3;
  const float* __restrict__ P = a.prep;
  const int L = a.L;
  const int npad = a.ntiles * PPL;
  const int SG = sg_total(HP, L);
  float* const partG = part + (size_t)grp * 4 * 12 * 32;
  float* const sink = sgacc + sg_wout(HP, L) + 3 * HP;
  for (int i = tid; i < SG; i += 2 * GT) sgacc[i] = 0.f;
  for (int i = tid; i < 3 * HP; i += 2 * GT) { woutL[i] = P[prep_wout(HP, L) + i]; w0L[i] = P[prep_w0x(HP) + i]; }
  __syncthreads();
  float lsum[4] = {0.f, 0.f, 0.f, 0.f};
  float dbo[3] = {0.f, 0.f, 0.f};

  SW sw(ldsb, P, woutL, w0L, w, lane0);

  auto bias = [&](int l) {
    return [&, l](int fb, int g, int, int h) {
      typedef __attribute__((address_space(4))) const f32x4 cf32x4;
      const cf32x4* bp = (const cf32x4*)(uintptr_t)(P + prep_b(HP, l) + sw.qbase(fb, g));
      const f32x4 b0 = bp[0], b1 = bp[1];
      return h ? b1 : b0;
    };
  };
  auto S_of = [&](int tile, int l) { return a.S + spill_off<act_block(HP, COLS)>(a.spill, tile, l, L); };
  auto Sw_of = [&](int tile, int l) { return fa.S + spill_off<act_block(HP, COLS)>(a.spill, tile, l, L); };
  auto Z_of = [&](int tile, int l) { return a.Zb + spill_off<act_block(HP, COLS)>(a.spill, tile, l, L); };
  auto none = [](auto&&...) {};

  auto point_stage = [&](int tile, int col, bool owner, float vtm_old, float (&oc)[3][4]) {
    const int pt = tile * PPL + col;
    const bool m = pt < a.n;
    float ov[3][4];
#pragma unroll
    for (int c3 = 0; c3 < 3; ++c3)
#pragma unroll
      for (int s = 0; s < 4; ++s) {
        float v = s == 0 ? P[prep_bout(HP, L) + c3] : 0.f;
#pragma unroll
        for (int ww = 0; ww < 4; ++ww) v += partG[(ww * 12 + c3 * 4 + s) * 32 + col];
        ov[c3][s] = v;
      }
    const float sc = fa.scale, sc2 = fa.scale * fa.scale;
    float u = ov[0][0], ux = ov[0][1] * sc, uy = ov[0][2] * sc, ud = ov[0][3] * sc2;
    float v = ov[1][0], vx = ov[1][1] * sc, vy = ov[1][2] * sc, vd = ov[1][3] * sc2;
    float p = ov[2][0], pxx = ov[2][1] * sc, pyy = ov[2][2] * sc;
    float vt = 0.f;
    float ev = (fa.e && m) ? fa.e[pt] : 0.f;
    if (fa.vtm && m) {
      vt = fminf(fa.vis_t0, vtm_old);
      if (owner) fa.vtm[pt] = fa.alpha_evm * fabsf(ev);
    }
    if (owner && fa.vis_used && m) fa.vis_used[pt] = vt;
    float nu = fa.inv_re + vt;
    float eq1 = (u * ux + v * uy) + pxx - nu * ud;
    float eq2 = (u * vx + v * vy) + pyy - nu * vd;
    float eq3 = ux + vy;
    float eq4 = fa.e ? (eq1 * (u - 0.5f) + eq2 * (v - 0.5f)) - ev : 0.f;
    if (owner) {
      float* f = fa.fld + pt;
      f[FLD_U * (size_t)npad] = u; f[FLD_V * (size_t)npad] = v;
      f[FLD_UX * (size_t)npad] = ux; f[FLD_UY * (size_t)npad] = uy;
      f[FLD_VX * (size_t)npad] = vx; f[FLD_VY * (size_t)npad] = vy;
      f[FLD_EQ1 * (size_t)npad] = eq1; f[FLD_EQ2 * (size_t)npad] = eq2;
      f[FLD_EQ3 * (size_t)npad] = eq3; f[FLD_EQ4 * (size_t)npad] = eq4;
      f[FLD_P * (size_t)npad] = p;
      if (m) {
        float ww = fa.w ? fa.w[pt] : 1.f;
        lsum[0] += ww * eq1 * eq1; lsum[1] += ww * eq2 * eq2;
        lsum[2] += ww * eq3 * eq3; lsum[3] += ww * eq4 * eq4;
      }
    }
    float ww = m ? (a.w ? a.w[pt] : 1.f) : 0.f;
    float g1 = a.coef_eq[0] * ww * eq1, g2 = a.coef_eq[1] * ww * eq2, g3 = a.coef_eq[2] * ww * eq3;
    float g4 = a.e ? a.coef_eq[3] * ww * eq4 : 0.f;
    float r1 = g1 + g4 * (u - 0.5f), r2 = g2 + g4 * (v - 0.5f), r3 = g3;
    float nub = a.inv_re + ((a.vis_used && m) ? vt : 0.f);
    const float bsc = a.scale, bsc2 = a.scale * a.scale;
    float au = r1 * ux + r2 * vx + g4 * eq1;
    float av = r1 * uy + r2 * vy + g4 * eq2;
    oc[0][0] = au; oc[0][1] = (r1 * u + r3) * bsc; oc[0][2] = (r1 * v) * bsc; oc[0][3] = -nub * r1 * bsc2;
    oc[1][0] = av; oc[1][1] = (r2 * u) * bsc; oc[1][2] = (r2 * v + r3) * bsc; oc[1][3] = -nub * r2 * bsc2;
    oc[2][0] = 0.f; oc[2][1] = r1 * bsc; oc[2][2] = r2 * bsc; oc[2][3] = 0.f;
#pragma unroll
    for (int c = 0; c < 3; ++c)
#pragma unroll
      for (int s = 0; s < 4; ++s) asm volatile("" : "+v"(oc[c][s]));
    if (owner) {
      if (a.ebar && m) a.ebar[pt] = -g4;
      dbo[0] += au; dbo[1] += av;
    }
  };

  auto seed = [&](int tile, float vtm_old) {
    return [&, tile, vtm_old](int col, int h, float (&oc)[3][4]) {
      if (tile < a.ntiles) {
        point_stage(tile, col, w == 0 && h == 0, vtm_old, oc);
      } else {
#pragma unroll
        for (int c = 0; c < 3; ++c)
#pragma unroll
          for (int s = 0; s < 4; ++s) { oc[c][s] = 0.f; asm volatile("" : "+v"(oc[c][s])); }
      }
    };
  };

  const int npairs = (a.ntiles + 1) / 2;
  if (grp == 1) SW::idle();
  for (int pair = blockIdx.x; pair < npairs; pair += gridDim.x) {
    const int tile = 2 * pair + grp;
    float px, py, vtm_old;
    {
      const int pt = tile * PPL + (lane0 & 31);
      px = pt < a.n ? a.x[pt] : 0.f; py = pt < a.n ? a.y[pt] : 0.f;
      vtm_old = (fa.vtm && pt < a.n) ? fa.vtm[pt] : 0.f;
    }
    sw.template fphase<0, true>(0, tile, nullptr, a.x, a.y, a.n, partG, bias(0), none);
    for (int l = 1; l < L - 1; ++l) {
      sw.template mphase<false, false>(l, nullptr);
      sw.template fphase<1, true>(l, tile, Sw_of(tile, l), a.x, a.y, a.n, partG, bias(l), none);
    }
    sw.template mphase<false, false>(L - 1, nullptr);
    sw.template fphase<2, true>(L - 1, tile, nullptr, a.x, a.y, a.n, partG, bias(L - 1), none);
    sw.template bphase<0, true>(L - 1, L, nullptr, Z_of(tile, L - 1), px, py, sgacc, sink, seed(tile, vtm_old), none);
    for (int l = L - 1; l >= 2; --l) {
      sw.template mphase<true, true>(l, S_of(tile, l - 1));
      sw.template bphase<1, true>(l - 1, L, S_of(tile, l - 1), Z_of(tile, l - 1), px, py, sgacc, sink, none, none);
    }
    sw.template mphase<true, false>(1, nullptr);
    sw.template bphase<2, true>(0, L, nullptr, Z_of(tile, 0), px, py, sgacc, sink, none, none);
  }
  if (grp == 0) SW::idle();
  float* red = reinterpret_cast<float*>(ldsb);
  __syncthreads();
#pragma unroll
  for (int k = 0; k < 4; ++k) red[k * 2 * GT + tid] = lsum[k];
  __syncthreads();
  if (tid < 4) {
    float s = 0.f;
    for (int t = 0; t < 2 * GT; ++t) s += red[tid * 2 * GT + t];
    fa.partials[blockIdx.x * PINN_NLOSS + tid] = s;
  } else if (tid < PINN_NLOSS) {
    fa.partials[blockIdx.x * PINN_NLOSS + tid] = 0.f;
  }
  __syncthreads();
#pragma unroll
  for (int c = 0; c < 3; ++c) red[c * 2 * GT + tid] = dbo[c];
  __syncthreads();
  if (tid < 3) {
    float s = 0.f;
    for (int t = 0; t < 2 * GT; ++t) s += red[tid * 2 * GT + t];
    sgacc[sg_bout(HP, L) + tid] = s;
  }
  __syncthreads();
  float* out = a.sg + (size_t)blockIdx.x * SG;
  for (int i = tid; i < SG; i += 2 * GT) out[i] = i >= sg_wout(HP, L) + 3 * HP && i < sg_bout(HP, L) ? 0.f : sgacc[i];
}

size_t fwdbwd_split_lds_bytes(int HP, int L) { (void)HP; return FusedLds<256>::bytes(L); }

template <int HP, int TERMS>
static int launch_one(const FwdArgs& fa, const BwdArgs& a, int grid, hipStream_t s) {
  const size_t lds = FusedLds<HP>::bytes(a.L);
  if (!spill_is(a.spill, act_block(HP), IN_P24_COMPACT) || !spill_is(fa.spill, act_block(HP), IN_P24_COMPACT)) return -1000;
  return launch_or_configure(&fwdbwd_split_kernel<HP, TERMS>, dim3(grid), dim3(2 * HP), lds, s, a.configure, fa, a);
}

int launch_fwdbwd_split(int HP, int terms, const FwdArgs& fa, const BwdArgs& a, int grid, hipStream_t s) {
  if (HP != 256) return -1000;
  return terms == 3 ? launch_one<256, 3>(fa, a, grid, s) : launch_one<256, 1>(fa, a, grid, s);
}
```

nsfnet_amd/csrc/kernels.h:

```cpp
#pragma once
#include <hip/hip_runtime.h>
#include <type_traits>
#include "fixed_fold.h"
#include "layout.h"
#include "spill.h"

typedef float f32x16 __attribute__((ext_vector_type(16)));
typedef float f32x4 __attribute__((ext_vector_type(4)));

#ifdef __HIPCC__
typedef __attribute__((address_space(1))) f32x4 gf32x4;
__device__ __forceinline__ gf32x4* pin_base(const void* q) {
  const unsigned long long b = (unsigned long long)q;
  const unsigned lo = __builtin_amdgcn_readfirstlane((unsigned)b), hi = __builtin_amdgcn_readfirstlane((unsigned)(b >> 32));
  return (gf32x4*)(((unsigned long long)hi << 32) | lo);
}
template <typename... Params, typename... Args>
static int launch_or_configure(void (*kernel)(Params...), dim3 grid, dim3 block, size_t lds, hipStream_t s, int configure,
                               const Args&... args) {
  if (configure)
    return -(int)hipFuncSetAttribute(reinterpret_cast<const void*>(kernel), hipFuncAttributeMaxDynamicSharedMemorySize, PINN_LDS_MAX);
  hipLaunchKernelGGL(kernel, grid, block, lds, s, args...);
  return -(int)hipGetLastError();
}
template <class F>
static int dispatch_ns_terms(int NS, int terms, F f) {
  using std::integral_constant;
  if (terms == 3) return NS == 4 ? f(integral_constant<int, 4>{}, integral_constant<int, 3>{}) : f(integral_constant<int, 1>{}, integral_constant<int, 3>{});
  return NS == 4 ? f(integral_constant<int, 4>{}, integral_constant<int, 1>{}) : f(integral_constant<int, 1>{}, integral_constant<int, 1>{});
}
#endif

enum { FLD_U = 0, FLD_V, FLD_UX, FLD_UY, FLD_VX, FLD_VY, FLD_EQ1, FLD_EQ2, FLD_EQ3, FLD_EQ4, FLD_P, FLD_COUNT };

struct HardBc { int kind, m; float x0, y0, inv_len, r, c; };

struct FwdArgs {
  const float* x; const float* y;
  int n;
  int ntiles;
  int L;
  int n_out;
  const float* prep;
  float* S;
  float* fld;
  const float* e;
  const float* w;
  float* vtm;
  float* vis_used;
  float inv_re, vis_t0, alpha_evm, scale;
  float* pred[3];
  const float* tgt[3];
  float* oadj;
  float coef[3];
  float* partials;
  int stagger;
  int configure;
  Spill spill;
  HardBc hbc;
};

struct BwdArgs {
  const float* x; const float* y;
  int n, ntiles, L, n_out;
  const float* prep;
  const float* S;
  float* Zb;
  const float* fld; const float* e; const float* w; const float* vis_used;
  float coef_eq[4];
  float inv_re, scale;
  float* ebar;
  const float* oadj;
  float* sg;
  int configure;
  Spill spill;
  HardBc hbc;
};

struct DwArgs {
  const float* S; const float* Zb;
  int ntiles, L, groups;
  float* slabs;
  int configure;
  const float* x; const float* y; const float* prep; int n;
  Spill spill;
};

struct ReduceSrc { const float* slabs; int groups; const float* sg; int nwg; };
struct ReduceArgs {
  ReduceSrc src[4]; int nsrc;
  int H, HP, L, n_out;
  float* grads; int accumulate;
};

struct ReduceLoc { int sgi; int layer; size_t slab_off; };
__device__ __forceinline__ ReduceLoc reduce_locate(size_t p, int H, int HP, int L, int n_out) {
  ReduceLoc r{-1, -1, 0};
  if (p < (size_t)2 * H) {
    int o = (int)(p / 2), j = (int)(p % 2);
    r.sgi = (j == 0 ? sg_w0x(HP, L) : sg_w0y(HP, L)) + o;
  } else if (p < (size_t)3 * H) {
    r.sgi = sg_db(HP, 0) + (int)(p - 2 * H);
  } else if (p < flat_w(H, L)) {
    size_t rel = p - (size_t)3 * H;
    size_t per = (size_t)H * H + H;
    int l = 1 + (int)(rel / per);
    size_t q = rel % per;
    if (q < (size_t)H * H) { r.layer = l; r.slab_off = (q / H) * HP + (q % H); }
    else r.sgi = sg_db(HP, l) + (int)(q - (size_t)H * H);
  } else {
    size_t q = p - flat_w(H, L);
    if (q < (size_t)n_out * H) r.sgi = sg_wout(HP, L) + (int)(q / H) * HP + (int)(q % H);
    else r.sgi = sg_bout(HP, L) + (int)(q - (size_t)n_out * H);
  }
  return r;
}
__device__ __forceinline__ double reduce_source_add(double s, const ReduceSrc& src, const ReduceLoc& loc, int HP,
                                                    size_t SG, int w) {
  const float* base; size_t stride; int n;
  if (loc.layer >= 0) { base = src.slabs + (size_t)(loc.layer - 1) * src.groups * HP * HP + loc.slab_off; stride = (size_t)HP * HP; n = src.groups; }
  else { base = src.sg + loc.sgi; stride = SG; n = src.nwg; }
  int g = w;
  for (; g + 24 < n; g += 32) {
    float v0 = base[(size_t)g * stride], v1 = base[(size_t)(g + 8) * stride];
    float v2 = base[(size_t)(g + 16) * stride], v3 = base[(size_t)(g + 24) * stride];
    s += (double)v0; s += (double)v1; s += (double)v2; s += (double)v3;
  }
  for (; g < n; g += 8) s += (double)base[(size_t)g * stride];
  return s;
}

struct TermReduceArgs {
  ReduceSrc src[4]; int nsrc[3];
  int H, HP, L, n_out;
  float* out[3]; int acc_mask;
  double* partials;
  double* gram;
};

__device__ __forceinline__ void wave_gram(float r, float b, float s, int lane, double* __restrict__ out) {
  const double dr = r, db = b, ds = s;
  double q[6] = {__dmul_rn(dr, dr), __dmul_rn(db, db), __dmul_rn(ds, ds),
                 __dmul_rn(dr, db), __dmul_rn(dr, ds), __dmul_rn(db, ds)};
#pragma unroll
  for (int c = 0; c < 6; ++c) q[c] = wave_fold<FoldSum>(q[c]);
  if (lane == 0) {
#pragma unroll
    for (int c = 0; c < 6; ++c) out[c] = q[c];
  }
}

int launch_fwd(int HP, int NS, const FwdArgs& a, int grid, hipStream_t s);
int launch_bwd(int HP, int NS, const BwdArgs& a, int grid, hipStream_t s);
int launch_dw(int HP, int NS, const DwArgs& a, hipStream_t s);
size_t fwd_lds_bytes(int HP);
size_t bwd_lds_bytes(int HP, int L);
size_t dw_lds_bytes(int HP);
int dw_threads(int HP);

int launch_prep(const float* params, float* prep, int H, int HP, int L, int n_out, int prec_fwd, int prec_bwd,
                hipStream_t s);
int launch_fwd_wide(int HP, int NS, const FwdArgs& a, int grid, hipStream_t s);
int launch_bwd_wide(int HP, int NS, const BwdArgs& a, int grid, hipStream_t s);
int launch_dw_wide(int HP, int NS, const DwArgs& a, hipStream_t s);
size_t fwd_wide_lds_bytes(int HP);
size_t bwd_wide_lds_bytes(int HP, int L);
size_t dw_wide_lds_bytes();
int launch_fwd_bf16(int HP, int NS, int terms, int cols, const FwdArgs& a, int grid, hipStream_t s);
int launch_bwd_bf16(int HP, int NS, int terms, int cols, const BwdArgs& a, int grid, hipStream_t s);
int launch_dw_bf16(int HP, int NS, int terms, int cols, const DwArgs& a, hipStream_t s);
size_t fwd_bf16_lds_bytes(int HP, int L, int cols);
size_t bwd_bf16_lds_bytes(int HP, int L, int cols);
size_t dw_bf16_lds_bytes(int HP);
int launch_fwd_bf16_wide(int HP, int NS, int terms, const FwdArgs& a, int grid, hipStream_t s);
int launch_bwd_bf16_wide(int HP, int NS, int terms, const BwdArgs& a, int grid, hipStream_t s);
int launch_dw_bf16_wide(int HP, int NS, int terms, const DwArgs& a, hipStream_t s);
size_t dw_bf16_wide_lds_bytes();
size_t fwd_bf16_wide_lds_bytes(int HP, int L);
size_t bwd_bf16_wide_lds_bytes(int HP, int L);
int launch_fwd_pipe(int HP, int terms, const FwdArgs& a, int grid, hipStream_t s);
size_t fwd_pipe_lds_bytes(int HP, int L);
int launch_fwd_split(int HP, int terms, const FwdArgs& a, int grid, hipStream_t s);
size_t fwd_split_lds_bytes(int HP, int L);
int launch_bwd_split(int HP, int terms, const BwdArgs& a, int grid, hipStream_t s);
size_t bwd_split_lds_bytes(int HP, int L);
int launch_fwdbwd_split(int HP, int terms, const FwdArgs& fa, const BwdArgs& a, int grid, hipStream_t s);
size_t fwdbwd_split_lds_bytes(int HP, int L);
int launch_bwd_pipe(int HP, int terms, const BwdArgs& a, int grid, hipStream_t s);
size_t bwd_pipe_lds_bytes(int HP, int L);
int launch_fwd_wsplit(int HP, int terms, const FwdArgs& a, int grid, hipStream_t s);
size_t fwd_wsplit_lds_bytes(int HP);
int launch_bwd_wsplit(int HP, int terms, const BwdArgs& a, int grid, hipStream_t s);
size_t bwd_wsplit_lds_bytes(int HP, int L);
int launch_reduce(const ReduceArgs& a, hipStream_t s);
int launch_loss_sums(const float* partials, int nparts, float* out, hipStream_t s);
int launch_adam_dev(float* p, const float* g, float* m, float* v, long n, float lr, float b1, float b2,
                    float eps, long long* step_counter, hipStream_t s);
int launch_adam(float* p, const float* g, float* m, float* v, long n, float step_size, float b1, float b2,
                float eps, float bc2_sqrt, hipStream_t s);
size_t resample_scratch_bytes(long n_pool);
int launch_resample_select(long n, const float* fields, long npad, double w4, double k, double c, double u, long m,
                           void* scratch, long long* out, hipStream_t s);
int launch_resample_gather(const long long* idx, long lo, long hi, long n_pool, const float* sx, const float* sy,
                           const float* sw, const float* sv, float* dx, float* dy, float* dw, float* dv, void* scratch,
                           double* w_sum, hipStream_t s);
size_t lbfgs_workspace_bytes(long n, long m);
int launch_lbfgs_reset(void* ws, long n, long m, hipStream_t s);
int launch_lbfgs_direction(void* ws, long n, long m, const float* g, float t_prev, float* d, double* result,
                           hipStream_t s);
int launch_lbfgs_probe(void* ws, long n, long m, const float* g, const float* d, double* result, hipStream_t s);
long balance_blocks(long n);
int launch_reduce_terms(const TermReduceArgs& a, hipStream_t s);
int launch_balance_stats(const float* v0, const float* v1, const float* v2, long n, double* partials, hipStream_t s);
int launch_balance_update(const double* partials, long n, int terms, double beta, float* lam, double* record,
                          hipStream_t s);
int launch_balance_combine(float* g, const float* gr, const float* gb, const float* gs, const float* lam, long n,
                           hipStream_t s);
int launch_confgrad_gram(const float* v0, const float* v1, const float* v2, long n, double* partials, hipStream_t s);
int launch_confgrad_coef(const double* partials, long n, int nterms, float* coef, double* record, hipStream_t s);
int launch_confgrad_combine(float* g, const float* gr, const float* gb, const float* gs, const float* coef, long n,
                            hipStream_t s);
struct BatchDrawArgs {
  long n, b;
  unsigned seed, rank;
  long long* counter;
  const float *sx, *sy, *sw, *sv;
  float *dx, *dy, *dw, *dv;
  long long* idx;
};
int launch_batch_draw(const BatchDrawArgs& a, hipStream_t s);
int launch_batch_scatter(const long long* idx, long b, long n, const float* src, float* dst, hipStream_t s);
struct RbaApplyArgs {
  long n, npad, n_store;
  const float* fld;
  double w4, gamma, eta;
  const long long* idx;
  const float* s;
  float *lam, *w;
  double *scratch, *record;
};
long rba_blocks(long n);
size_t rba_scratch_bytes(long n);
int launch_rba_stats(long n, const float* fld, long npad, double w4, double* scratch, hipStream_t s);
int launch_rba_apply(const RbaApplyArgs& a, hipStream_t s);
int launch_rba_fill(long n, double init, const float* sw, float* lam, float* w, hipStream_t s);
constexpr int VAL_RECORD = 8, VAL_STATE = 8;
struct ValStatsArgs {
  const float* pred[3];
  const float* tgt[3];
  long n, capacity;
  int metric;
  double t, every;
  double *scratch, *state, *ring;
};
struct ValKeepArgs {
  const float* src[2];
  float* dst[2];
  long n[2];
  const double* state;
};
size_t val_scratch_bytes();
int launch_val_stats(const ValStatsArgs& a, hipStream_t s);
int launch_val_keep(const ValKeepArgs& a, hipStream_t s);
```

nsfnet_amd/csrc/layout.h:

```cpp
#pragma once
#include <stddef.h>
#include <stdint.h>

#ifdef __HIPCC__
#define PINN_HD __host__ __device__ __forceinline__
#else
#define PINN_HD inline
#endif

#define PINN_TILE_COLS 128
#define PINN_MAX_HP 512
#define PINN_NLOSS 8
#define PINN_LDS_MAX 163840

PINN_HD size_t prep_w0x(int HP) { (void)HP; return 0; }
PINN_HD size_t prep_w0y(int HP) { return (size_t)HP; }
PINN_HD size_t prep_b0(int HP) { return (size_t)2 * HP; }
PINN_HD size_t prep_layer_stride(int HP) { return (size_t)2 * HP * HP + HP; }
PINN_HD size_t prep_wf(int HP, int l) { return (size_t)3 * HP + (size_t)(l - 1) * prep_layer_stride(HP); }
PINN_HD size_t prep_wtf(int HP, int l) { return prep_wf(HP, l) + (size_t)HP * HP; }
PINN_HD size_t prep_b(int HP, int l) { return prep_wf(HP, l) + (size_t)2 * HP * HP; }
PINN_HD size_t prep_wout(int HP, int L) { return (size_t)3 * HP + (size_t)(L - 1) * prep_layer_stride(HP); }
PINN_HD size_t prep_bout(int HP, int L) { return prep_wout(HP, L) + (size_t)4 * HP; }
PINN_HD size_t prep_total(int HP, int L) { return prep_bout(HP, L) + 4; }

PINN_HD int sg_db(int HP, int l) { return l * HP; }
PINN_HD int sg_w0x(int HP, int L) { return L * HP; }
PINN_HD int sg_w0y(int HP, int L) { return L * HP + HP; }
PINN_HD int sg_wout(int HP, int L) { return L * HP + 2 * HP; }
PINN_HD int sg_bout(int HP, int L) { return L * HP + 6 * HP; }
PINN_HD int sg_total(int HP, int L) { return L * HP + 6 * HP + 4; }

PINN_HD int mfma_row(int r, int h) { return (r & 3) + 8 * (r >> 2) + 4 * h; }

PINN_HD constexpr size_t act_block(int HP, int cols = PINN_TILE_COLS) { return (size_t)HP * cols; }

PINN_HD size_t flat_w(int H, int l) { return l == 0 ? 0 : (size_t)3 * H + (size_t)(l - 1) * ((size_t)H * H + H); }
PINN_HD size_t flat_b(int H, int l, int L, int n_out) {
  (void)n_out;
  return flat_w(H, l) + (l == 0 ? (size_t)2 * H : (l == L ? (size_t)n_out * H : (size_t)H * H));
}
PINN_HD size_t flat_total(int H, int L, int n_out) { return flat_b(H, L, L, n_out) + n_out; }
```

nsfnet_amd/csrc/misc.hip:

```cpp
#include "kernels.h"
#include "optim.h"

__device__ __forceinline__ unsigned short f2bf_rne(float x) {
  return __builtin_bit_cast(unsigned short, (__bf16)x);
}

__device__ __forceinline__ unsigned short bf16_frag_elem(const float* W, int H, int HP, bool tr, int pos, int lo_part) {
  int j = pos & 7, lane = (pos >> 3) & 63, ws = pos >> 9;
  int KS = HP / 16, s = ws % KS, w = ws / KS;
  int k = 16 * s + 8 * (lane >> 5) + j, o = 32 * w + (lane & 31);
  float v = 0.f;
  if (o < H && k < H) v = tr ? W[(size_t)k * H + o] : W[(size_t)o * H + k];
  unsigned short hi = f2bf_rne(v);
  if (!lo_part) return hi;
  return f2bf_rne(v - __uint_as_float(((unsigned)hi) << 16));
}

__global__ void prep_kernel(const float* __restrict__ params, float* __restrict__ prep,
                            int H, int HP, int L, int n_out, int prec_fwd, int prec_bwd) {
  const size_t total = prep_total(HP, L);
  for (size_t idx = blockIdx.x * (size_t)blockDim.x + threadIdx.x; idx < total;
       idx += (size_t)gridDim.x * blockDim.x) {
    float v = 0.f;
    if (idx < (size_t)3 * HP) {
      int which = (int)(idx / HP), o = (int)(idx % HP);
      if (o < H) v = which == 0 ? params[flat_w(H, 0) + 2 * o] : which == 1 ? params[flat_w(H, 0) + 2 * o + 1]
                                                                            : params[flat_b(H, 0, L, n_out) + o];
    } else if (idx < prep_wout(HP, L)) {
      size_t rel = idx - (size_t)3 * HP;
      int l = 1 + (int)(rel / prep_layer_stride(HP));
      size_t q = rel % prep_layer_stride(HP);
      const float* W = params + flat_w(H, l);
      if (q < (size_t)2 * HP * HP) {
        bool tr = q >= (size_t)HP * HP;
        size_t f = tr ? q - (size_t)HP * HP : q;
        if ((tr ? prec_bwd : prec_fwd) != 0) {
          int e0 = (int)(2 * f), half = HP * HP;
          unsigned short b0 = bf16_frag_elem(W, H, HP, tr, e0 % half, e0 / half);
          unsigned short b1 = bf16_frag_elem(W, H, HP, tr, (e0 + 1) % half, (e0 + 1) / half);
          prep[idx] = __uint_as_float((unsigned)b0 | ((unsigned)b1 << 16));
          continue;
        }
        int e = (int)(f & 3), lane = (int)((f >> 2) & 63);
        int wq = (int)(f >> 8);
        int qq = wq % (HP / 8), w = wq / (HP / 8);
        int k = 2 * (4 * qq + e) + (lane >> 5), o = 32 * w + (lane & 31);
        if (o < H && k < H) v = tr ? W[(size_t)k * H + o] : W[(size_t)o * H + k];
      } else {
        int o = (int)(q - (size_t)2 * HP * HP);
        if (o < H) v = params[flat_b(H, l, L, n_out) + o];
      }
    } else if (idx < prep_bout(HP, L)) {
      size_t q = idx - prep_wout(HP, L);
      int c = (int)(q / HP), k = (int)(q % HP);
      if (c < n_out && k < H) v = params[flat_w(H, L) + (size_t)c * H + k];
    } else {
      int c = (int)(idx - prep_bout(HP, L));
      if (c < n_out) v = params[flat_b(H, L, L, n_out) + c];
    }
    prep[idx] = v;
  }
}

int launch_prep(const float* params, float* prep, int H, int HP, int L, int n_out, int prec_fwd, int prec_bwd,
                hipStream_t s) {
  size_t total = prep_total(HP, L);
  int blocks = (int)((total + 255) / 256);
  if (blocks > 4096) blocks = 4096;
  hipLaunchKernelGGL(prep_kernel, dim3(blocks), dim3(256), 0, s, params, prep, H, HP, L, n_out, prec_fwd, prec_bwd);
  return launch_status();
}

__global__ __launch_bounds__(512) void reduce_kernel(ReduceArgs a) {
  __shared__ double part[8][64];
  const int H = a.H, HP = a.HP, L = a.L;
  const size_t P = flat_total(H, L, a.n_out);
  const int lane = threadIdx.x & 63, w = threadIdx.x >> 6;
  const size_t p = blockIdx.x * (size_t)64 + lane;
  const bool live = p < P;
  const ReduceLoc loc = live ? reduce_locate(p, H, HP, L, a.n_out) : ReduceLoc{-1, -1, 0};
  double s = 0.0;
  if (live) {
    const size_t SG = sg_total(HP, L);
    for (int k = 0; k < a.nsrc; ++k) s = reduce_source_add(s, a.src[k], loc, HP, SG, w);
  }
  part[w][lane] = s;
  __syncthreads();
  if (w == 0 && live) {
    double t = part[0][lane];
#pragma unroll
    for (int i = 1; i < 8; ++i) t += part[i][lane];
    if (a.accumulate) a.grads[p] += (float)t; else a.grads[p] = (float)t;
  }
}

int launch_reduce(const ReduceArgs& a, hipStream_t s) {
  size_t P = flat_total(a.H, a.L, a.n_out);
  hipLaunchKernelGGL(reduce_kernel, dim3((unsigned)((P + 63) / 64)), dim3(512), 0, s, a);
  return launch_status();
}

__global__ __launch_bounds__(256) void loss_sums_kernel(const float* __restrict__ partials, int nparts, float* __restrict__ out) {
  __shared__ double part[32][PINN_NLOSS];
  const int k = threadIdx.x % PINN_NLOSS, j = threadIdx.x / PINN_NLOSS;
  double s = 0.0;
  for (int i = j; i < nparts; i += 32) s += (double)partials[(size_t)i * PINN_NLOSS + k];
  part[j][k] = s;
  __syncthreads();
  if (threadIdx.x < PINN_NLOSS) {
    double t = part[0][k];
    for (int i = 1; i < 32; ++i) t += part[i][k];
    out[k] = (float)t;
  }
}

int launch_loss_sums(const float* partials, int nparts, float* out, hipStream_t s) {
  static_assert(PINN_NLOSS * 32 == 256, "loss_sums_kernel layout");
  hipLaunchKernelGGL(loss_sums_kernel, dim3(1), dim3(256), 0, s, partials, nparts, out);
  return launch_status();
}

__global__ void adam_kernel(float* __restrict__ p, const float* __restrict__ g, float* __restrict__ m,
                            float* __restrict__ v, long n, float step_size, float b1, float b2, float eps,
                            float bc2_sqrt) {
  adam_update<false>(p, g, m, v, blockIdx.x * (long)blockDim.x + threadIdx.x, (long)gridDim.x * blockDim.x,
                      n, step_size, b1, b2, eps, bc2_sqrt);
}

__global__ void adam_dev_kernel(float* __restrict__ p, const float* __restrict__ g, float* __restrict__ m,
                                float* __restrict__ v, long n, float lr, float b1, float b2, float eps,
                                long long* step_counter) {
  float step_size, bc2_sqrt;
  adam_bias_correction(lr, b1, b2, step_counter, step_size, bc2_sqrt);
  adam_update<false>(p, g, m, v, blockIdx.x * (long)blockDim.x + threadIdx.x, (long)gridDim.x * blockDim.x,
                      n, step_size, b1, b2, eps, bc2_sqrt);
  __syncthreads();
  if (threadIdx.x == 0 && last_ticket(step_counter + 1)) step_counter[0] = step_counter[0] + 1;
}

int launch_adam_dev(float* p, const float* g, float* m, float* v, long n, float lr, float b1, float b2,
                    float eps, long long* step_counter, hipStream_t s) {
  if (n <= 0) return 0;
  int blocks = (int)((n + 255) / 256);
  if (blocks > 2048) blocks = 2048;
  hipLaunchKernelGGL(adam_dev_kernel, dim3(blocks), dim3(256), 0, s, p, g, m, v, n, lr, b1, b2, eps, step_counter);
  return launch_status();
}

int launch_adam(float* p, const float* g, float* m, float* v, long n, float step_size, float b1, float b2,
                float eps, float bc2_sqrt, hipStream_t s) {
  if (n <= 0) return 0;
  int blocks = (int)((n + 255) / 256);
  if (blocks > 2048) blocks = 2048;
  hipLaunchKernelGGL(adam_kernel, dim3(blocks), dim3(256), 0, s, p, g, m, v, n, step_size, b1, b2, eps, bc2_sqrt);
  return launch_status();
}
```

nsfnet_amd/csrc/split_phases.h:

```cpp
#pragma once
#include "kernels.h"
#include "bf16_util.h"
#include "reduce_util.h"

template <int HP, int TERMS>
struct SplitWave {
  static_assert(HP == 256, "four waves x 64 features per group");
  using XI = XImg<HP, 32>;
  typedef __attribute__((address_space(1))) u32x4 gu32x4;
  static constexpr int KS = HP / 16, PPL = 32, COLS = 128;
  static constexpr int RING = 2, WPRE = RING - 1;
  static constexpr int SQ = 2;
  static constexpr size_t PLQ = (size_t)(HP / 4) * PPL;

  unsigned char* const X;
  const float* const P;
  const float* const woutL;
  const float* const w0L;
  const int w, lane0;
  f32x16 acc[2][4];
  u32x2 st[2][4][2];
  u32x4 wh[2][RING], wl[2][RING];
  u32x4 sq[SQ + 1][3];
  u32x4 skeep[8][3];
  bool have_parked = false;

  __device__ __forceinline__ SplitWave(unsigned char* X_, const float* P_, const float* woutL_, const float* w0L_, int w_, int lane0_)
      : X(X_), P(P_), woutL(woutL_), w0L(w0L_), w(w_), lane0(lane0_) {}

  __device__ __forceinline__ int phase_lane() const {
    int lane = lane0;
    asm volatile("" : "+v"(lane));
    return lane;
  }
  __device__ __forceinline__ int qbase(int fb, int g) const { return 64 * (2 * fb + (g >> 1)) + 16 * w + 8 * (g & 1); }
  __device__ __forceinline__ int quad_o(int qq, int h) const { return qbase(qq >> 2, qq & 3) + 4 * h; }
  __device__ __forceinline__ int w_lane(int col, int h) const {
    return ((2 * (col >> 4) + (w >> 1)) * KS) * 64 + 16 * (w & 1) + (col & 15) + 32 * h;
  }
  __device__ __forceinline__ void wload(size_t poff, int s, int wlane) {
    const gu32x4* const wf = reinterpret_cast<const gu32x4*>(pin_base(reinterpret_cast<const u32x4*>(P + poff)));
#pragma unroll
    for (int fb = 0; fb < 2; ++fb) {
      wh[fb][s % RING] = (wf + (size_t)fb * 4 * KS * 64 + s * 64)[wlane];
      if (TERMS == 3) wl[fb][s % RING] = (wf + (size_t)(HP * HP / 8) + (size_t)fb * 4 * KS * 64 + s * 64)[wlane];
    }
  }
  __device__ __forceinline__ void dump_kp(int fb, int g0, int k, int p, int col, int h) {
    const int off = XI::chunk_off(col, qbase(fb, g0 + k) >> 3) + 8 * h;
    *reinterpret_cast<u32x2*>(X + p * XI::PLANE * 2 + off) = st[k][p][0];
    if (TERMS == 3) *reinterpret_cast<u32x2*>(X + XI::HALF * 2 + p * XI::PLANE * 2 + off) = st[k][p][1];
  }
  __device__ __forceinline__ void dump_k(int fb, int g0, int k, int col, int h) {
#pragma unroll
    for (int p = 0; p < 4; ++p) dump_kp(fb, g0, k, p, col, h);
  }
  __device__ __forceinline__ void dump(int fb, int g0, int col, int h) { dump_k(fb, g0, 0, col, h); dump_k(fb, g0, 1, col, h); }
  __device__ __forceinline__ void sload(const float* Sl, int qq, int col, int h) {
    const int o = quad_o(qq, h);
    const unsigned so = (unsigned)(((o - 4 * h) >> 2) + h) * PPL + col;
#pragma unroll
    for (int k = 0; k < 3; ++k)
      sq[qq % (SQ + 1)][k] = __builtin_bit_cast(u32x4, __builtin_nontemporal_load(pin_base(reinterpret_cast<const f32x4*>(Sl) + k * PLQ) + so));
  }
  __device__ __forceinline__ static void idle() {
#pragma unroll
    for (int q = 0; q < 4; ++q) __syncthreads();
  }

  template <bool REV, bool PRE_S>
  __device__ __forceinline__ void mphase(int l, const float* Snext) {
    const int lane = phase_lane(), col = lane & 31, h = lane >> 5;
    const int wlane = w_lane(col, h);
    const size_t poff = REV ? prep_wtf(HP, l) : prep_wf(HP, l);
    u32x4 bh[2], bo[2];
    auto bload = [&](int u) {
      const int s = u >> 2, j = u & 3;
      const int off = XI::chunk_off(col, 2 * s + h);
      bh[u & 1] = *reinterpret_cast<const u32x4*>(X + j * XI::PLANE * 2 + off);
      if (TERMS == 3) bo[u & 1] = *reinterpret_cast<const u32x4*>(X + XI::HALF * 2 + j * XI::PLANE * 2 + off);
    };
#pragma unroll
    for (int q = 0; q < 4; ++q) {
      if (REV && q == 0 && have_parked) dump(1, 2, col, h);
      bload(16 * q);
#pragma unroll
      for (int u = 16 * q; u < 16 * q + 16; ++u) {
        const int s = u >> 2, j = u & 3;
        if (j == 0 && s + WPRE < KS) wload(poff, s + WPRE, wlane);
        if (PRE_S && u >= 4 * (KS - WPRE) && u < 4 * (KS - WPRE) + SQ) sload(Snext, u - 4 * (KS - WPRE), col, h);
        if ((u & 15) != 15) bload(u + 1);
        if (!REV && q == 0 && (u & 1)) dump_kp(1, 2, u >> 3, (u >> 1) & 3, col, h);
#pragma unroll
        for (int fb = 0; fb < 2; ++fb) {
          if (s == 0) {
            const f32x16 zero = {0.f, 0.f, 0.f, 0.f, 0.f, 0.f, 0.f, 0.f, 0.f, 0.f, 0.f, 0.f, 0.f, 0.f, 0.f, 0.f};
            acc[fb][j] = TERMS == 3 ? mfma_bf16(wh[fb][0], bo[u & 1], zero) : mfma_bf16(wh[fb][0], bh[u & 1], zero);
            if (TERMS == 3) {
              acc[fb][j] = mfma_bf16(wl[fb][0], bh[u & 1], acc[fb][j]);
              acc[fb][j] = mfma_bf16(wh[fb][0], bh[u & 1], acc[fb][j]);
            }
          } else {
            if (TERMS == 3) {
              acc[fb][j] = mfma_bf16(wh[fb][s % RING], bo[u & 1], acc[fb][j]);
              acc[fb][j] = mfma_bf16(wl[fb][s % RING], bh[u & 1], acc[fb][j]);
            }
            acc[fb][j] = mfma_bf16(wh[fb][s % RING], bh[u & 1], acc[fb][j]);
          }
        }
        __builtin_amdgcn_sched_barrier(0);
      }
      __syncthreads();
    }
    have_parked = false;
  }

  template <int EK, bool KEEP, class Bias, class Quarter>
  __device__ __forceinline__ void fphase(int lE, int tileE, float* Sl, const float* x, const float* y, int n, float* partG,
                                         Bias bias, Quarter quarter) {
    constexpr bool last = EK == 2, first = EK == 0;
    const int lane = phase_lane(), col = lane & 31, h = lane >> 5;
    float po[3][4];
#pragma unroll
    for (int c = 0; c < 3; ++c)
#pragma unroll
      for (int s = 0; s < 4; ++s) po[c][s] = 0.f;
    float px = 0.f, py = 0.f;
    if (first) {
      const int pt = tileE * PPL + col;
      px = pt < n ? x[pt] : 0.f; py = pt < n ? y[pt] : 0.f;
    }
#pragma unroll
    for (int q = 0; q < 4; ++q) {
      quarter(q);
      const int fb = q >> 1;
#pragma unroll
      for (int k = 0; k < 2; ++k) {
        const int g = 2 * (q & 1) + k, o = qbase(fb, g) + 4 * h;
        if (!last && q == 3 && k == 1) {
#pragma unroll
          for (int s = 0; s < WPRE; ++s) wload(prep_wf(HP, lE + 1), s, w_lane(col, h));
        }
        f32x4 av[4], sv[4];
        f32x4 b4, wx4, wy4;
        if (first) {
          wx4 = *reinterpret_cast<const f32x4*>(w0L + o); wy4 = *reinterpret_cast<const f32x4*>(w0L + HP + o);
          b4 = *reinterpret_cast<const f32x4*>(w0L + 2 * HP + o);
        } else {
          b4 = bias(fb, g, o, h);
        }
#pragma unroll
        for (int e = 0; e < 4; ++e) {
          const int r = 4 * g + e;
          float z, zx, zy, zd;
          if (first) {
            z = layer0_z(wx4[e], wy4[e], b4[e], px, py); zx = wx4[e]; zy = wy4[e]; zd = 0.f;
          } else {
            z = acc[fb][0][r] + b4[e]; zx = acc[fb][1][r]; zy = acc[fb][2][r]; zd = acc[fb][3][r];
          }
          const float t = fast_tanh(z);
          const float d1 = 1.f - t * t;
          const float d2 = -2.f * t * d1;
          av[0][e] = t; av[1][e] = d1 * zx; av[2][e] = d1 * zy; av[3][e] = d2 * (zx * zx + zy * zy) + d1 * zd;
          sv[0][e] = t; sv[1][e] = zx; sv[2][e] = zy; sv[3][e] = zd;
          __builtin_amdgcn_sched_barrier(0);
        }
        const unsigned so = (unsigned)(((o - 4 * h) >> 2) + h) * PPL + col;
        u32x4 pk[3];
        if (q > 0 && !last) dump_k((q - 1) >> 1, 2 * ((q - 1) & 1), k, col, h);
#pragma unroll
        for (int p = 0; p < 4; ++p) {
          if (!last) {
            split4(av[p][0], av[p][1], av[p][2], av[p][3], st[k][p][0], st[k][p][1]);
          } else {
#pragma unroll
            for (int c = 0; c < 3; ++c) {
              const f32x4 wo = *reinterpret_cast<const f32x4*>(woutL + c * HP + o);
#pragma unroll
              for (int e = 0; e < 4; ++e) po[c][p] = fmaf(wo[e], av[p][e], po[c][p]);
            }
          }
          if (!first) {
            pack24_plane(sv[p], p, pk);
            if (!(KEEP && last)) store24_planes(Sl, PLQ, so, p, pk);
          }
          if (last) asm volatile("" : "+v"(po[0][p]), "+v"(po[1][p]), "+v"(po[2][p]));
          __builtin_amdgcn_sched_barrier(0);
        }
        if (KEEP && last) {
#pragma unroll
          for (int kk = 0; kk < 3; ++kk) skeep[2 * q + k][kk] = pk[kk];
        }
        __builtin_amdgcn_sched_barrier(0);
      }
      if (last && q == 3) {
#pragma unroll
        for (int c = 0; c < 3; ++c)
#pragma unroll
          for (int s = 0; s < 4; ++s)
            partG[(w * 12 + c * 4 + s) * 32 + col] = po[c][s] + __shfl_xor(po[c][s], 32, 64);
      }
      __syncthreads();
    }
  }

  template <int EK, bool KEEP, class Seed, class Quarter>
  __device__ __forceinline__ void bphase(int lE, int L, const float* Sl, float* Zl, float pxE, float pyE, float* sgacc,
                                         float* sink, Seed seed, Quarter quarter) {
    constexpr bool first = EK == 0, last = EK == 2;
    const int lane = phase_lane(), col = lane & 31, h = lane >> 5;
    float oc[3][4];
    if (first) seed(col, h, oc);
    auto commit = [&](int base, int o4, float v) {
      float* p = col < 4 ? &sgacc[base + o4 + (col & 3)] : &sink[lane];
      lds_rmw_add(p, v);
    };
    if (first && !KEEP) {
#pragma unroll
      for (int qq = 0; qq < SQ; ++qq) sload(Sl, qq, col, h);
    }
#pragma unroll
    for (int q = 0; q < 4; ++q) {
      if (q > 0 && !last) dump((q - 1) >> 1, 2 * ((q - 1) & 1), col, h);
      const int fb = q >> 1;
#pragma unroll
      for (int k = 0; k < 2; ++k) {
        const int g = 2 * (q & 1) + k, qq = 2 * q + k, o = quad_o(qq, h);
        if (!last && !(first && KEEP) && qq + SQ < 8) sload(Sl, qq + SQ, col, h);
        if (!last && qq == 7) {
#pragma unroll
          for (int s = 0; s < WPRE; ++s) wload(prep_wtf(HP, lE), s, w_lane(col, h));
        }
        f32x4 sc[4];
        if (last) {
          layer0_saved(*reinterpret_cast<const f32x4*>(w0L + o), *reinterpret_cast<const f32x4*>(w0L + HP + o),
                       *reinterpret_cast<const f32x4*>(w0L + 2 * HP + o), pxE, pyE, TanhFast(), sc[0], sc[1], sc[2], sc[3]);
        } else if (first && KEEP) {
#pragma unroll
          for (int p = 0; p < 4; ++p) {
            sc[p] = unpack24_plane(skeep[qq], p);
            asm volatile("" : "+v"(sc[p]));
          }
        } else {
#pragma unroll
          for (int p = 0; p < 4; ++p) sc[p] = unpack24_plane(sq[qq % (SQ + 1)], p);
        }
        f32x4 zq[4], wov[3], dwv[2], wo4[3];
        if (first) {
#pragma unroll
          for (int c = 0; c < 3; ++c) wo4[c] = *reinterpret_cast<const f32x4*>(woutL + c * HP + o);
        }
#pragma unroll
        for (int e = 0; e < 4; ++e) {
          const int r = 4 * g + e;
          float ga, gx, gy, gd;
          if (first) {
            ga = wo4[0][e] * oc[0][0] + wo4[1][e] * oc[1][0] + wo4[2][e] * oc[2][0];
            gx = wo4[0][e] * oc[0][1] + wo4[1][e] * oc[1][1] + wo4[2][e] * oc[2][1];
            gy = wo4[0][e] * oc[0][2] + wo4[1][e] * oc[1][2] + wo4[2][e] * oc[2][2];
            gd = wo4[0][e] * oc[0][3] + wo4[1][e] * oc[1][3] + wo4[2][e] * oc[2][3];
          } else {
            ga = acc[fb][0][r]; gx = acc[fb][1][r]; gy = acc[fb][2][r]; gd = acc[fb][3][r];
          }
          const float t = sc[0][e], zx = sc[1][e], zy = sc[2][e], zd = sc[3][e];
          const float d1 = 1.f - t * t;
          const float d2 = -2.f * t * d1;
          const float d3 = -2.f * d1 * (1.f - 3.f * t * t);
          const float zz = zx * zx + zy * zy;
          zq[1][e] = d1 * gx + 2.f * d2 * zx * gd;
          zq[2][e] = d1 * gy + 2.f * d2 * zy * gd;
          zq[3][e] = d1 * gd;
          zq[0][e] = d1 * ga + d2 * (zx * gx + zy * gy) + (d3 * zz + d2 * zd) * gd;
          if (first) {
            const float ax = d1 * zx, ay = d1 * zy, ad = fmaf(d1, zd, d2 * zz);
#pragma unroll
            for (int c = 0; c < 3; ++c) wov[c][e] = fmaf(oc[c][3], ad, fmaf(oc[c][2], ay, fmaf(oc[c][0], t, oc[c][1] * ax)));
          }
          if (last) { dwv[0][e] = zq[0][e] * pxE + zq[1][e]; dwv[1][e] = zq[0][e] * pyE + zq[2][e]; }
          __builtin_amdgcn_sched_barrier(0);
        }
        commit(sg_db(HP, lE), o, sum_cols4<32>(zq[0][0], zq[0][1], zq[0][2], zq[0][3], lane));
        if (first) {
#pragma unroll
          for (int c = 0; c < 3; ++c)
            commit(sg_wout(HP, L) + c * HP, o, sum_cols4<32>(wov[c][0], wov[c][1], wov[c][2], wov[c][3], lane));
        }
        if (last) {
          commit(sg_w0x(HP, L), o, sum_cols4<32>(dwv[0][0], dwv[0][1], dwv[0][2], dwv[0][3], lane));
          commit(sg_w0y(HP, L), o, sum_cols4<32>(dwv[1][0], dwv[1][1], dwv[1][2], dwv[1][3], lane));
        }
        __builtin_amdgcn_sched_barrier(0);
        if (!last) {
          const unsigned so = (unsigned)(((o - 4 * h) >> 2) + h) * PPL + col;
          u32x4 pk[3];
#pragma unroll
          for (int p = 0; p < 4; ++p) {
            split4(zq[p][0], zq[p][1], zq[p][2], zq[p][3], st[k][p][0], st[k][p][1]);
            pack24_plane(zq[p], p, pk);
            store24_planes(Zl, PLQ, so, p, pk);
            __builtin_amdgcn_sched_barrier(0);
          }
        }
        __builtin_amdgcn_sched_barrier(0);
      }
      quarter(q);
      __syncthreads();
    }
    have_parked = !last;
  }
};
```

Measured before the change: 43.38 million.

## Sum hidden-layer bias gradients inside dW kernel instead of backward phase

```diff
diff --git a/nsfnet_amd/csrc/balance.hip b/nsfnet_amd/csrc/balance.hip
--- a/nsfnet_amd/csrc/balance.hip
+++ b/nsfnet_amd/csrc/balance.hip
@@ -20,7 +20,7 @@
   const int lane = threadIdx.x & 63, w = threadIdx.x >> 6;
   const size_t p = blockIdx.x * (size_t)64 + lane;
   const bool live = p < P;
-  const ReduceLoc loc = live ? reduce_locate(p, H, HP, L, a.n_out) : ReduceLoc{-1, -1, 0};
+  const ReduceLoc loc = live ? reduce_locate(p, H, HP, L, a.n_out) : ReduceLoc{-1, -1, 0, 0, 0};
   const size_t SG = sg_total(HP, L);
   int k = 0;
   for (int t = 0; t < 3; ++t) {
diff --git a/nsfnet_amd/csrc/bwd_bf16_split.hip b/nsfnet_amd/csrc/bwd_bf16_split.hip
--- a/nsfnet_amd/csrc/bwd_bf16_split.hip
+++ b/nsfnet_amd/csrc/bwd_bf16_split.hip
@@ -11,7 +11,7 @@
   static size_t bytes(int L) { return X_BYTES + (OADJ_F + DUMMY_F + 6 * HP + (size_t)sg_total(HP, L)) * sizeof(float); }
 };
 
-template <int HP, int TERMS>
+template <int HP, int TERMS, bool DBDW>
 __global__ __launch_bounds__(2 * HP, 1) void bwd_split_kernel(BwdArgs a) {
   using G = SplitBwdLds<HP>;
   using SW = SplitWave<HP, TERMS>;
@@ -66,13 +66,13 @@
   for (int pair = blockIdx.x; pair < npairs; pair += gridDim.x) {
     const int tile = 2 * pair + grp;
     const int next_tile = pair + (int)gridDim.x < npairs ? 2 * (pair + (int)gridDim.x) + grp : -1;
-    sw.template bphase<0, false>(L - 1, L, S_of(tile, L - 1), Z_of(tile, L - 1), px, py, sgacc, dummy + wave * 64, oadj, none);
+    sw.template bphase<0, false, DBDW>(L - 1, L, S_of(tile, L - 1), Z_of(tile, L - 1), px, py, sgacc, dummy + wave * 64, oadj, none);
     for (int l = L - 1; l >= 2; --l) {
       sw.template mphase<true, true>(l, S_of(tile, l - 1));
-      sw.template bphase<1, false>(l - 1, L, S_of(tile, l - 1), Z_of(tile, l - 1), px, py, sgacc, dummy + wave * 64, oadj, none);
+      sw.template bphase<1, false, DBDW>(l - 1, L, S_of(tile, l - 1), Z_of(tile, l - 1), px, py, sgacc, dummy + wave * 64, oadj, none);
     }
     sw.template mphase<true, false>(1, nullptr);
-    sw.template bphase<2, false>(0, L, S_of(tile, 0), Z_of(tile, 0), px, py, sgacc, dummy + wave * 64, oadj,
+    sw.template bphase<2, false, DBDW>(0, L, S_of(tile, 0), Z_of(tile, 0), px, py, sgacc, dummy + wave * 64, oadj,
                                  [&](int q) { if (q == 3 && next_tile >= 0) seeds(next_tile, pxN, pyN); });
     px = pxN; py = pyN;
   }
@@ -98,7 +98,8 @@
 static int launch_one(const BwdArgs& a, int grid, hipStream_t s) {
   const size_t lds = SplitBwdLds<HP>::bytes(a.L);
   if (!spill_is(a.spill, act_block(HP), IN_P24_COMPACT)) return -1000;
-  return launch_or_configure(&bwd_split_kernel<HP, TERMS>, dim3(grid), dim3(2 * HP), lds, s, a.configure, a);
+  if (a.db_dw) return launch_or_configure(&bwd_split_kernel<HP, TERMS, true>, dim3(grid), dim3(2 * HP), lds, s, a.configure, a);
+  return launch_or_configure(&bwd_split_kernel<HP, TERMS, false>, dim3(grid), dim3(2 * HP), lds, s, a.configure, a);
 }
 
 int launch_bwd_split(int HP, int terms, const BwdArgs& a, int grid, hipStream_t s) {
diff --git a/nsfnet_amd/csrc/capi.hip b/nsfnet_amd/csrc/capi.hip
--- a/nsfnet_amd/csrc/capi.hip
+++ b/nsfnet_amd/csrc/capi.hip
@@ -28,6 +28,7 @@
   int s0_skip32;
   int verbose;
   int tile_cols;
+  int db_dw;
 };
 static int env_int(const char* name, int dflt) {
   const char* v = getenv(name);
@@ -37,7 +38,7 @@
   const int sched = env_int("PINN_SCHED", 2);
   return {env_int("PINN_FWD_SCHED", sched), env_int("PINN_BWD_SCHED", sched), env_int("PINN_WSPLIT", 1),
           env_int("PINN_FUSE", 1), env_int("PINN_STAGGER", 0), env_int("PINN_S0_SKIP32", 1),
-          env_int("PINN_VERBOSE", 0), env_int("PINN_TILE_COLS", 0)};
+          env_int("PINN_VERBOSE", 0), env_int("PINN_TILE_COLS", 0), env_int("PINN_DB_DW", 1)};
 }
 
 struct pinn_net_s {
@@ -101,7 +102,8 @@
   Role role[ROLE_COUNT];
   Spill spill;
   HardBc hbc;
-  size_t off_partials, off_oadj, off_sg, off_slabs, off_S, off_Zb, bytes_fwd, bytes_all;
+  int db_dw;
+  size_t off_partials, off_oadj, off_sg, off_slabs, off_dbw, off_S, off_Zb, bytes_fwd, bytes_all;
 };
 
 static int num_cus() {
@@ -166,6 +168,7 @@
   const pinn_net_s& n = plan->net;
   const Role& r = plan->role[ROLE_BWD];
   const int NS = plan->streams, terms = terms_of(n.prec_bwd);
+  if (a.db_dw && r.family != FAM_SPLIT) return -1000;
   switch (r.family) {
     case FAM_FP32: return launch_bwd(n.HP, NS, a, r.grid, s);
     case FAM_FP32_WIDE: return launch_bwd_wide(n.HP, NS, a, r.grid, s);
@@ -180,6 +183,7 @@
 static int run_dw(const pinn_plan_s* plan, const DwArgs& d, hipStream_t s) {
   const pinn_net_s& n = plan->net;
   const int NS = plan->streams, terms = terms_of(n.prec_dw);
+  if (d.db_dw != plan->db_dw || (d.db_dw && plan->role[ROLE_DW].family != FAM_BF16)) return -1000;
   switch (plan->role[ROLE_DW].family) {
     case FAM_FP32: return launch_dw(n.HP, NS, d, s);
     case FAM_FP32_WIDE: return launch_dw_wide(n.HP, NS, d, s);
@@ -189,6 +193,7 @@
   }
 }
 static int run_fused(const pinn_plan_s* plan, const FwdArgs& fa, const BwdArgs& ba, hipStream_t s) {
+  if (ba.db_dw != plan->db_dw) return -1000;
   return launch_fwdbwd_split(plan->net.HP, terms_of(plan->net.prec_fwd), fa, ba, plan->role[ROLE_FUSED].grid, s);
 }
 
@@ -278,6 +283,14 @@
   p->off_S = off;        off = align_up(off + (size_t)(p->ntiles + 1) * spill_tile * 4, 256);
   p->off_Zb = off;       off = align_up(off + (size_t)(p->ntiles + 1) * spill_tile * 4, 256);
   p->bytes_all = off;
+  p->off_dbw = p->off_Zb + (size_t)p->ntiles * spill_tile * 4;
+  p->db_dw = split_pair && sw.db_dw != 0 && p->groups > 0 && dbw_total(HP, p->groups, L) <= spill_tile;
+  if (p->db_dw && !(p->role[ROLE_BWD].family == FAM_SPLIT && p->role[ROLE_DW].family == FAM_BF16 &&
+                    spill_is(p->spill, ablk, IN_P24_COMPACT)))
+    return fail(-5, "pinn_plan_create: internal error: db summed in dW outside the role-split plan%s");
+  if (sw.verbose && split_pair)
+    fprintf(stderr, "[pinn] plan: role-split pair, fused sweeps %d (%zu bytes of LDS), hidden-layer db summed in dW %d\n",
+            (int)fuse, fwdbwd_split_lds_bytes(HP, L), p->db_dw);
   return 0;
 }
 
@@ -313,6 +326,7 @@
   a.sg = WS(plan, off_sg);
   a.spill = plan->spill;
   a.hbc = plan->hbc;
+  a.db_dw = plan->db_dw;
   return a;
 }
 static BwdArgs residual_bwd_args(const pinn_plan_s* plan, void* ws, const float* prep, const float* x, const float* y,
@@ -332,6 +346,7 @@
   d.slabs = WS(plan, off_slabs);
   d.x = x; d.y = y; d.prep = prep; d.n = (int)plan->n;
   d.spill = plan->spill;
+  d.db_dw = plan->db_dw; d.dbw = plan->db_dw ? WS(plan, off_dbw) : nullptr;
   return d;
 }
 
@@ -564,6 +579,7 @@
       return fail(-22, "%s: plan belongs to a different net", who);
     src[k].slabs = WS(p, off_slabs); src[k].groups = p->groups;
     src[k].sg = WS(p, off_sg); src[k].nwg = p->role[ROLE_BWD].grid;
+    src[k].dbw = p->db_dw ? WS(p, off_dbw) : nullptr;
   }
   return 0;
 }
diff --git a/nsfnet_amd/csrc/dw_bf16.hip b/nsfnet_amd/csrc/dw_bf16.hip
--- a/nsfnet_amd/csrc/dw_bf16.hip
+++ b/nsfnet_amd/csrc/dw_bf16.hip
@@ -1,5 +1,6 @@
 #include "kernels.h"
 #include "bf16_util.h"
+#include "reduce_util.h"
 
 template <int T> struct DwCfgB;
 template <> struct DwCfgB<1> { static constexpr int TM = 1, TN = 1; };
@@ -27,12 +28,13 @@
   return __builtin_bit_cast(u32x2, v);
 }
 
-template <int HP, int NS, int TERMS, int PPL, bool REC, bool P24>
+template <int HP, int NS, int TERMS, int PPL, bool REC, bool P24, bool DBW>
 __device__ __forceinline__ void dw_bf16_body(const DwArgs& a) {
   constexpr int CPT = PPL / 8;
   constexpr size_t ABLK = act_block(HP, 4 * PPL);
   using DI = DwImg<HP>;
   static_assert(P24 || !REC, "no fp32-format reader that recomputes layer 0");
+  static_assert(P24 || !DBW, "db is summed from the 24-bit z-bars only");
   constexpr int T = HP / 32;
   constexpr int TM = DwCfgB<T>::TM, TN = DwCfgB<T>::TN;
   constexpr int WN = T / TN;
@@ -61,6 +63,7 @@
     wx4 = w0[og]; wy4 = w0[HP / 4 + og]; b4 = w0[2 * (HP / 4) + og];
   }
   f32x4 zrA[4], srA[4];
+  f32x4 dbacc = {0.f, 0.f, 0.f, 0.f};
   struct Raw24 { u32x4 z[3], s[3]; float px, py; };
   Raw24 rawA, rawB;
   auto gload24 = [&](int ch, Raw24& R) {
@@ -93,6 +96,7 @@
         zr[s] = unpack24(u32x2{R.z[s >> 1][2 * (s & 1)], R.z[s >> 1][2 * (s & 1) + 1]}, R.z[2][s]);
         if (!rec) sr[s] = unpack24(u32x2{R.s[s >> 1][2 * (s & 1)], R.s[s >> 1][2 * (s & 1) + 1]}, R.s[2][s]);
       }
+      if (DBW) dbacc += zr[0];
     }
     f32x4 av[4];
     if (rec) {
@@ -225,6 +229,18 @@
   if (nch > 0) mfma_chunk((nch - 1) & 1);
   __syncthreads();
   }
+  if (DBW) {
+    f32x4 d;
+#pragma unroll
+    for (int e = 0; e < 4; ++e) {
+      float v = dbacc[e];
+      v += dpp_mov<0xB1>(v);
+      v += dpp_mov<0x4E>(v);
+      v += dpp_mov<0x141>(v);
+      d[e] = v;
+    }
+    if (p == 0) *reinterpret_cast<f32x4*>(a.dbw + dbw_off(HP, a.groups, l, g) + 4 * og) = d;
+  }
   float* slab = a.slabs + ((size_t)(l - 1) * a.groups + g) * HP * HP;
 #pragma unroll
   for (int m = 0; m < TM; ++m)
@@ -238,10 +254,10 @@
       }
 }
 
-template <int HP, int NS, int TERMS, int PPL, bool P24, bool REC0>
+template <int HP, int NS, int TERMS, int PPL, bool P24, bool REC0, bool DBW = false>
 __global__ __launch_bounds__(HP * 2) void dw_bf16_kernel(DwArgs a) {
-  if (REC0 && blockIdx.y == 0) dw_bf16_body<HP, NS, TERMS, PPL, REC0, P24>(a);
-  else dw_bf16_body<HP, NS, TERMS, PPL, false, P24>(a);
+  if (REC0 && blockIdx.y == 0) dw_bf16_body<HP, NS, TERMS, PPL, REC0, P24, DBW>(a);
+  else dw_bf16_body<HP, NS, TERMS, PPL, false, P24, DBW>(a);
 }
 
 template <int HP>
@@ -255,10 +271,10 @@
   }
 }
 
-template <int HP, int NS, int TERMS, int PPL, bool P24, bool REC0>
+template <int HP, int NS, int TERMS, int PPL, bool P24, bool REC0, bool DBW = false>
 static int launch_fmt(const DwArgs& a, hipStream_t s) {
   size_t lds = lds_bytes_t<HP>();
-  return launch_or_configure(&dw_bf16_kernel<HP, NS, TERMS, PPL, P24, REC0>, dim3(a.groups, a.L - 1), dim3(HP * 2), lds, s, a.configure, a);
+  return launch_or_configure(&dw_bf16_kernel<HP, NS, TERMS, PPL, P24, REC0, DBW>, dim3(a.groups, a.L - 1), dim3(HP * 2), lds, s, a.configure, a);
 }
 template <int HP, int NS, int TERMS, int PPL>
 static int launch_one(const DwArgs& a, hipStream_t s) {
@@ -266,9 +282,10 @@
   if (!spill_is(a.spill, act_block(HP, 4 * PPL), CAN_COMPACT ? IN_CLASSIC | IN_P24_COMPACT : IN_CLASSIC)) return -1000;
   const bool p24 = a.spill.quad == SPILL_QUAD_P24, rec0 = a.spill.skip0 != 0;
   if constexpr (CAN_COMPACT) {
+    if (p24 && rec0 && a.db_dw) return a.dbw || a.configure ? launch_fmt<HP, NS, TERMS, PPL, true, true, true>(a, s) : -1000;
     if (p24 && rec0) return launch_fmt<HP, NS, TERMS, PPL, true, true>(a, s);
   }
-  return p24 || rec0 ? -1000 : launch_fmt<HP, NS, TERMS, PPL, false, false>(a, s);
+  return p24 || rec0 || a.db_dw ? -1000 : launch_fmt<HP, NS, TERMS, PPL, false, false>(a, s);
 }
 
 template <int HP, int PPL>
diff --git a/nsfnet_amd/csrc/fwdbwd_bf16_split.hip b/nsfnet_amd/csrc/fwdbwd_bf16_split.hip
--- a/nsfnet_amd/csrc/fwdbwd_bf16_split.hip
+++ b/nsfnet_amd/csrc/fwdbwd_bf16_split.hip
@@ -9,7 +9,7 @@
   static size_t bytes(int L) { return X_BYTES + (PART_F + 6 * HP + (size_t)sg_total(HP, L)) * sizeof(float); }
 };
 
-template <int HP, int TERMS>
+template <int HP, int TERMS, bool DBDW>
 __global__ __launch_bounds__(2 * HP, 1) void fwdbwd_split_kernel(FwdArgs fa, BwdArgs a) {
   using G = FusedLds<HP>;
   using SW = SplitWave<HP, TERMS>;
@@ -28,7 +28,7 @@
   const int SG = sg_total(HP, L);
   float* const partG = part + (size_t)grp * 4 * 12 * 32;
   float* const sink = sgacc + sg_wout(HP, L) + 3 * HP;
-  for (int i = tid; i < SG; i += 2 * GT) sgacc[i] = 0.f;
+  for (int i = tid; i < SG; i += 2 * GT) sgacc[i] = DBDW && i >= HP && i < L * HP ? P[prep_b(HP, i / HP) + (i % HP)] : 0.f;
   for (int i = tid; i < 3 * HP; i += 2 * GT) { woutL[i] = P[prep_wout(HP, L) + i]; w0L[i] = P[prep_w0x(HP) + i]; }
   __syncthreads();
   float lsum[4] = {0.f, 0.f, 0.f, 0.f};
@@ -37,7 +37,8 @@
   SW sw(ldsb, P, woutL, w0L, w, lane0);
 
   auto bias = [&](int l) {
-    return [&, l](int fb, int g, int, int h) {
+    return [&, l](int fb, int g, int o, int h) {
+      if constexpr (DBDW) return *reinterpret_cast<const f32x4*>(sgacc + sg_bias_row(HP, l) + o);
       typedef __attribute__((address_space(4))) const f32x4 cf32x4;
       const cf32x4* bp = (const cf32x4*)(uintptr_t)(P + prep_b(HP, l) + sw.qbase(fb, g));
       const f32x4 b0 = bp[0], b1 = bp[1];
@@ -143,13 +144,13 @@
     }
     sw.template mphase<false, false>(L - 1, nullptr);
     sw.template fphase<2, true>(L - 1, tile, nullptr, a.x, a.y, a.n, partG, bias(L - 1), none);
-    sw.template bphase<0, true>(L - 1, L, nullptr, Z_of(tile, L - 1), px, py, sgacc, sink, seed(tile, vtm_old), none);
+    sw.template bphase<0, true, DBDW>(L - 1, L, nullptr, Z_of(tile, L - 1), px, py, sgacc, sink, seed(tile, vtm_old), none);
     for (int l = L - 1; l >= 2; --l) {
       sw.template mphase<true, true>(l, S_of(tile, l - 1));
-      sw.template bphase<1, true>(l - 1, L, S_of(tile, l - 1), Z_of(tile, l - 1), px, py, sgacc, sink, none, none);
+      sw.template bphase<1, true, DBDW>(l - 1, L, S_of(tile, l - 1), Z_of(tile, l - 1), px, py, sgacc, sink, none, none);
     }
     sw.template mphase<true, false>(1, nullptr);
-    sw.template bphase<2, true>(0, L, nullptr, Z_of(tile, 0), px, py, sgacc, sink, none, none);
+    sw.template bphase<2, true, DBDW>(0, L, nullptr, Z_of(tile, 0), px, py, sgacc, sink, none, none);
   }
   if (grp == 0) SW::idle();
   float* red = reinterpret_cast<float*>(ldsb);
@@ -175,7 +176,8 @@
   }
   __syncthreads();
   float* out = a.sg + (size_t)blockIdx.x * SG;
-  for (int i = tid; i < SG; i += 2 * GT) out[i] = i >= sg_wout(HP, L) + 3 * HP && i < sg_bout(HP, L) ? 0.f : sgacc[i];
+  for (int i = tid; i < SG; i += 2 * GT)
+    out[i] = (i >= sg_wout(HP, L) + 3 * HP && i < sg_bout(HP, L)) || (DBDW && i >= HP && i < L * HP) ? 0.f : sgacc[i];
 }
 
 size_t fwdbwd_split_lds_bytes(int HP, int L) { (void)HP; return FusedLds<256>::bytes(L); }
@@ -184,7 +186,8 @@
 static int launch_one(const FwdArgs& fa, const BwdArgs& a, int grid, hipStream_t s) {
   const size_t lds = FusedLds<HP>::bytes(a.L);
   if (!spill_is(a.spill, act_block(HP), IN_P24_COMPACT) || !spill_is(fa.spill, act_block(HP), IN_P24_COMPACT)) return -1000;
-  return launch_or_configure(&fwdbwd_split_kernel<HP, TERMS>, dim3(grid), dim3(2 * HP), lds, s, a.configure, fa, a);
+  if (a.db_dw) return launch_or_configure(&fwdbwd_split_kernel<HP, TERMS, true>, dim3(grid), dim3(2 * HP), lds, s, a.configure, fa, a);
+  return launch_or_configure(&fwdbwd_split_kernel<HP, TERMS, false>, dim3(grid), dim3(2 * HP), lds, s, a.configure, fa, a);
 }
 
 int launch_fwdbwd_split(int HP, int terms, const FwdArgs& fa, const BwdArgs& a, int grid, hipStream_t s) {
diff --git a/nsfnet_amd/csrc/kernels.h b/nsfnet_amd/csrc/kernels.h
--- a/nsfnet_amd/csrc/kernels.h
+++ b/nsfnet_amd/csrc/kernels.h
@@ -75,6 +75,7 @@
   int configure;
   Spill spill;
   HardBc hbc;
+  int db_dw;
 };
 
 struct DwArgs {
@@ -84,18 +85,19 @@
   int configure;
   const float* x; const float* y; const float* prep; int n;
   Spill spill;
-};
-
-struct ReduceSrc { const float* slabs; int groups; const float* sg; int nwg; };
+  int db_dw; float* dbw;
+};
+
+struct ReduceSrc { const float* slabs; int groups; const float* sg; int nwg; const float* dbw; };
 struct ReduceArgs {
   ReduceSrc src[4]; int nsrc;
   int H, HP, L, n_out;
   float* grads; int accumulate;
 };
 
-struct ReduceLoc { int sgi; int layer; size_t slab_off; };
+struct ReduceLoc { int sgi; int layer; size_t slab_off; int dbl; int dbo; };
 __device__ __forceinline__ ReduceLoc reduce_locate(size_t p, int H, int HP, int L, int n_out) {
-  ReduceLoc r{-1, -1, 0};
+  ReduceLoc r{-1, -1, 0, 0, 0};
   if (p < (size_t)2 * H) {
     int o = (int)(p / 2), j = (int)(p % 2);
     r.sgi = (j == 0 ? sg_w0x(HP, L) : sg_w0y(HP, L)) + o;
@@ -107,7 +109,7 @@
     int l = 1 + (int)(rel / per);
     size_t q = rel % per;
     if (q < (size_t)H * H) { r.layer = l; r.slab_off = (q / H) * HP + (q % H); }
-    else r.sgi = sg_db(HP, l) + (int)(q - (size_t)H * H);
+    else { r.dbl = l; r.dbo = (int)(q - (size_t)H * H); r.sgi = sg_db(HP, l) + r.dbo; }
   } else {
     size_t q = p - flat_w(H, L);
     if (q < (size_t)n_out * H) r.sgi = sg_wout(HP, L) + (int)(q / H) * HP + (int)(q % H);
@@ -119,6 +121,11 @@
                                                     size_t SG, int w) {
   const float* base; size_t stride; int n;
   if (loc.layer >= 0) { base = src.slabs + (size_t)(loc.layer - 1) * src.groups * HP * HP + loc.slab_off; stride = (size_t)HP * HP; n = src.groups; }
+  else if (loc.dbl >= 1 && src.dbw) {
+    base = src.dbw + dbw_off(HP, src.groups, loc.dbl, 0) + loc.dbo;
+    for (int g = w; g < src.groups; g += 8) s = FoldSum::apply(s, (double)base[(size_t)g * HP]);
+    return s;
+  }
   else { base = src.sg + loc.sgi; stride = SG; n = src.nwg; }
   int g = w;
   for (; g + 24 < n; g += 32) {
diff --git a/nsfnet_amd/csrc/layout.h b/nsfnet_amd/csrc/layout.h
--- a/nsfnet_amd/csrc/layout.h
+++ b/nsfnet_amd/csrc/layout.h
@@ -30,6 +30,9 @@
 PINN_HD int sg_wout(int HP, int L) { return L * HP + 2 * HP; }
 PINN_HD int sg_bout(int HP, int L) { return L * HP + 6 * HP; }
 PINN_HD int sg_total(int HP, int L) { return L * HP + 6 * HP + 4; }
+PINN_HD int sg_bias_row(int HP, int l) { return sg_db(HP, l); }
+PINN_HD size_t dbw_off(int HP, int groups, int l, int g) { return ((size_t)(l - 1) * groups + g) * HP; }
+PINN_HD size_t dbw_total(int HP, int groups, int L) { return (size_t)(L - 1) * groups * HP; }
 
 PINN_HD int mfma_row(int r, int h) { return (r & 3) + 8 * (r >> 2) + 4 * h; }
 
diff --git a/nsfnet_amd/csrc/misc.hip b/nsfnet_amd/csrc/misc.hip
--- a/nsfnet_amd/csrc/misc.hip
+++ b/nsfnet_amd/csrc/misc.hip
@@ -78,7 +78,7 @@
   const int lane = threadIdx.x & 63, w = threadIdx.x >> 6;
   const size_t p = blockIdx.x * (size_t)64 + lane;
   const bool live = p < P;
-  const ReduceLoc loc = live ? reduce_locate(p, H, HP, L, a.n_out) : ReduceLoc{-1, -1, 0};
+  const ReduceLoc loc = live ? reduce_locate(p, H, HP, L, a.n_out) : ReduceLoc{-1, -1, 0, 0, 0};
   double s = 0.0;
   if (live) {
     const size_t SG = sg_total(HP, L);
diff --git a/nsfnet_amd/csrc/split_phases.h b/nsfnet_amd/csrc/split_phases.h
--- a/nsfnet_amd/csrc/split_phases.h
+++ b/nsfnet_amd/csrc/split_phases.h
@@ -204,7 +204,7 @@
     }
   }
 
-  template <int EK, bool KEEP, class Seed, class Quarter>
+  template <int EK, bool KEEP, bool DBDW, class Seed, class Quarter>
   __device__ __forceinline__ void bphase(int lE, int L, const float* Sl, float* Zl, float pxE, float pyE, float* sgacc,
                                          float* sink, Seed seed, Quarter quarter) {
     constexpr bool first = EK == 0, last = EK == 2;
@@ -279,7 +279,7 @@
           if (last) { dwv[0][e] = zq[0][e] * pxE + zq[1][e]; dwv[1][e] = zq[0][e] * pyE + zq[2][e]; }
           __builtin_amdgcn_sched_barrier(0);
         }
-        commit(sg_db(HP, lE), o, sum_cols4<32>(zq[0][0], zq[0][1], zq[0][2], zq[0][3], lane));
+        if (last || !DBDW) commit(sg_db(HP, lE), o, sum_cols4<32>(zq[0][0], zq[0][1], zq[0][2], zq[0][3], lane));
         if (first) {
 #pragma unroll
           for (int c = 0; c < 3; ++c)
```

Result: no change. 43.44 million (median of 6 runs) (+0.1%).
